# lh3/miniprot

Hardware: NVIDIA H100
Metric: proteins/s (higher is better)
Workload: dtype int16 scores

## Files before the change

miniprot_b200/csrc/cuda/chain_core.cuh:

```cuda
#pragma once
#include <stdint.h>
#include "../flagsort.hpp"

#ifdef __CUDACC__
#define CHN_HD __host__ __device__ __forceinline__
#else
#define CHN_HD inline
#endif

namespace chn {

struct Par { int32_t max_dist_x, max_dist_y, bw, max_skip, max_iter, min_cnt, min_sc; float chn_coef_log; int32_t is_spliced, kmer, bbit; };

CHN_HD Par normalise(Par p)
{
	if (p.max_dist_x < p.bw) p.max_dist_x = p.bw;
	if (p.max_dist_y < p.bw && !p.is_spliced) p.max_dist_y = p.bw;
	return p;
}

CHN_HD float log2_approx(float x)
{
	union { float f; uint32_t i; } z;
	z.f = x;
	float r = (float)((int)((z.i >> 23) & 255) - 128);
	z.i &= ~(255u << 23);
	z.i += 127u << 23;
#ifdef __CUDA_ARCH__
	float q = __fadd_rn(__fmul_rn(-0.34484843f, z.f), 2.02466578f);
	q = __fsub_rn(__fmul_rn(q, z.f), 0.67487759f);
	return __fadd_rn(r, q);
#else
	volatile float q = -0.34484843f * z.f;
	q = q + 2.02466578f;
	q = q * z.f;
	q = q - 0.67487759f;
	volatile float s = r + q;
	return s;
#endif
}

CHN_HD int32_t pair_score(const Par &p, uint64_t ai, uint64_t aj)
{
	const int32_t dq = (int32_t)ai - (int32_t)aj, dq3 = dq * 3;
	int32_t dr3, dd, dds = 0, sc;
	if (dq <= 0 || dq3 > p.max_dist_x || dq > p.max_dist_y) return INT32_MIN;
	if (p.bbit > 0) {
		const int32_t bs = 1 << p.bbit;
		dr3 = (int32_t)(((ai >> 32) - (aj >> 32)) << p.bbit);
		if (dq3 < dr3 - bs) dd = dr3 - bs - dq3, dds = -dd;
		else if (dq3 > dr3 + bs) dd = dq3 - (dr3 + bs), dds = dd;
		else dd = 0;
	} else {
		dr3 = (int32_t)((ai >> 32) - (aj >> 32));
		if (dr3 == 0) return INT32_MIN;
		dd = dr3 > dq3 ? dr3 - dq3 : dq3 - dr3;
		dds = dq3 - dr3;
	}
	if (dd > p.bw) return INT32_MIN;
	if (p.bbit > 0) sc = p.kmer < dq ? p.kmer : dq;
	else if (p.kmer <= dq && p.kmer * 3 <= dr3) sc = p.kmer;
	else {
		const int32_t dr = dr3 / 3, g = dr < dq ? dr : dq;
		sc = g < p.kmer ? g : p.kmer;
		if (dr3 - dr * 3 != 0) --sc;
	}
	if (dd > 0) {
#ifdef __CUDA_ARCH__
		const float lin = __fmul_rn((float)dd, .33334f);
		const float lg = dd >= 2 ? __fadd_rn(__fmul_rn(p.chn_coef_log, __fsub_rn(log2_approx((float)(dd + 1)), 1.0f)), 1.0f) : (float)dd;
		if (p.is_spliced && dds < 0) sc -= (int32_t)(lin < lg ? lin : lg);
		else sc -= (int32_t)__fadd_rn(lin, lg);
#else
		volatile float lin = (float)dd * .33334f;
		volatile float lg = (float)dd;
		if (dd >= 2) { volatile float t = log2_approx((float)(dd + 1)) - 1.0f; t = p.chn_coef_log * t; lg = t + 1.0f; }
		if (p.is_spliced && dds < 0) sc -= (int32_t)(lin < lg ? lin : lg);
		else { volatile float s = lin + lg; sc -= (int32_t)s; }
#endif
	}
	if (p.bbit > 0 && ai >> 32 == aj >> 32 && dd == 0) sc += 2;
	return sc;
}

CHN_HD int resolve_chunk(uint32_t rec, uint32_t skip, int32_t max_skip, int32_t &n_skip)
{
	if (skip == 0) {
		const int32_t d = (int32_t)
#ifdef __CUDA_ARCH__
			__popc(rec);
#else
			__builtin_popcount(rec);
#endif
		n_skip = n_skip > d ? n_skip - d : 0;
		return 32;
	}
	uint32_t m = rec | skip;
	while (m) {
#ifdef __CUDA_ARCH__
		const int b = __ffs(m) - 1;
#else
		const int b = __builtin_ctz(m);
#endif
		if (rec >> b & 1) { if (n_skip > 0) --n_skip; }
		else if (++n_skip > max_skip) return b;
		m &= m - 1;
	}
	return 32;
}

CHN_HD uint64_t rec_key(uint64_t r) { return r >> 32; }

template <class T, class FT, class PT>
CHN_HD int64_t bk_end(int32_t max_drop, uint64_t z, const FT *f, const PT *p, T *t)
{
	const int32_t zx = (int32_t)(z >> 32);
	int64_t i = (int64_t)(uint32_t)z, end_i = -1, max_i = i;
	int32_t max_s = 0;
	if (i < 0 || t[i] != 0) return i;
	do {
		t[i] = 2;
		end_i = i = p[i];
		const int32_t s = i < 0 ? zx : zx - (int32_t)f[i];
		if (s > max_s) max_s = s, max_i = i;
		else if (max_s - s > max_drop) break;
	} while (i >= 0 && t[i] == 0);
	for (i = (int64_t)(uint32_t)z; i >= 0 && i != end_i; i = p[i]) t[i] = 0;
	return max_i;
}

template <class T, bool PRESORTED = false, class FT = int32_t, class PT = int32_t>
CHN_HD int32_t peel_chains(const Par &p, int32_t n_z, const FT *f, const PT *pp, T *t, int32_t *v, uint64_t *z, mpb::FlagRange<uint64_t> *stack, uint64_t *u,
                           int32_t *n_v_out = 0)
{
	const int32_t max_drop = p.is_spliced ? INT32_MAX : p.bw;
	int32_t n_u = 0, n_v = 0;
	if (n_v_out) *n_v_out = 0;
	if (n_z == 0) return 0;
	if (!PRESORTED) mpb::flag_sort_by(z, z + n_z, [](const uint64_t &e) { return rec_key(e); }, stack);
	for (int32_t k = n_z - 1; k >= 0; --k) {
		const int32_t zi = (int32_t)(uint32_t)z[k], zx = (int32_t)(z[k] >> 32);
		if (zx <= p.kmer && p.min_cnt >= 2) break;
		if (t[zi] != 0) continue;
		const int32_t n_v0 = n_v;
		const int64_t end_i = bk_end(max_drop, z[k], f, pp, t);
		int64_t i;
		for (i = zi; i != end_i; i = pp[i]) v[n_v++] = (int32_t)i, t[i] = 1;
		const int32_t sc = i < 0 ? zx : zx - (int32_t)f[i];
		if (sc >= p.min_sc && n_v > n_v0 && n_v - n_v0 >= p.min_cnt) u[n_u++] = (uint64_t)sc << 32 | (uint64_t)(n_v - n_v0);
		else n_v = n_v0;
	}
	if (n_v_out) *n_v_out = n_v;
	return n_u;
}

template <class FT, class Sync>
CHN_HD void compact_chains(int32_t n_u, const uint64_t *a, FT *f, const int32_t *v, uint64_t *z, mpb::FlagRange<uint64_t> *stack, uint64_t *u, uint64_t *b,
                           int32_t *n_b_out, int lane, int n_lanes, Sync sync)
{
	if (n_u == 0) {
		if (lane == 0) *n_b_out = 0;
		return;
	}
	if (lane == 0) {
		int32_t k = 0;
		for (int32_t i = 0; i < n_u; ++i) {
			const int32_t ni = (int32_t)(uint32_t)u[i];
			z[i] = (a[v[k + ni - 1]] >> 32) << 32 | (uint32_t)i;
			f[i] = (FT)k;
			k += ni;
		}
		mpb::flag_sort_by(z, z + n_u, [](const uint64_t &e) { return rec_key(e); }, stack);
	}
	sync();
	int32_t o = 0;
	for (int32_t i = 0; i < n_u; ++i) {
		const int32_t src = (int32_t)(uint32_t)z[i], k0 = (int32_t)f[src], ni = (int32_t)(uint32_t)u[src];
		for (int32_t j = lane; j < ni; j += n_lanes) b[o + j] = a[v[k0 + (ni - j - 1)]];
		o += ni;
	}
	sync();
	for (int32_t i = lane; i < n_u; i += n_lanes) z[i] = u[(uint32_t)z[i]];
	sync();
	for (int32_t i = lane; i < n_u; i += n_lanes) u[i] = z[i];
	if (lane == 0) *n_b_out = o;
}

template <class T, bool PRESORTED = false, class FT = int32_t, class PT = int32_t>
CHN_HD int32_t peel_and_compact(const Par &p, int32_t n_z, const uint64_t *a, FT *f, const PT *pp, T *t, int32_t *v, uint64_t *z,
                                mpb::FlagRange<uint64_t> *stack, uint64_t *u, uint64_t *b, int32_t *n_b_out)
{
	const int32_t n_u = peel_chains<T, PRESORTED, FT, PT>(p, n_z, f, pp, t, v, z, stack, u);
	compact_chains(n_u, a, f, v, z, stack, u, b, n_b_out, 0, 1, [] {});
	return n_u;
}

template <class T>
CHN_HD int32_t backtrack_compact(const Par &p, int32_t n, const uint64_t *a, int32_t *f, const int32_t *pp, T *t, int32_t *v, uint64_t *z,
                                 mpb::FlagRange<uint64_t> *stack, uint64_t *u, uint64_t *b, int32_t *n_b_out)
{
	int32_t n_z = 0;
	for (int32_t i = 0; i < n; ++i) {
		t[i] = 0;
		if (f[i] >= p.min_sc) z[n_z++] = (uint64_t)(uint32_t)f[i] << 32 | (uint32_t)i;
	}
	return peel_and_compact(p, n_z, a, f, pp, t, v, z, stack, u, b, n_b_out);
}

}
```

miniprot_b200/csrc/cuda/chain_dev.hpp:

```cpp
#pragma once
#include <cuda_runtime.h>
#include <stdint.h>
#include "chain_core.cuh"

namespace mpb {
namespace cuda {

constexpr int CHAIN_STACK = 2048;

void chain_launch_fill(cudaStream_t st, const int32_t *list, const int64_t *a_off, const int32_t *cnt, const uint64_t *a, int n_prob, const chn::Par &par, int32_t *f,
                       int32_t *p, int32_t *t);
void chain_launch_smem(cudaStream_t st, const int32_t *list, int n_list, int cap, const int64_t *a_off, const int32_t *cnt, const uint64_t *a, const chn::Par &par,
                       int32_t *v, void *stack, uint64_t *u, uint64_t *b, int32_t *n_u, int32_t *n_b, int resort);
void chain_launch_bt_smem(cudaStream_t st, const int32_t *list, int n_list, int cap, const int64_t *a_off, const int32_t *cnt, const uint64_t *a, const chn::Par &par,
                          int32_t *f, const int32_t *p, int32_t *v, void *stack, uint64_t *u, uint64_t *b, int32_t *n_u, int32_t *n_b, int resort);
void chain_launch_bt(cudaStream_t st, const int32_t *list, int n_list, const int64_t *a_off, const int32_t *cnt, const uint64_t *a, const chn::Par &par, int32_t *f,
                     const int32_t *p, int32_t *t, int32_t *v, void *z, void *stack, uint64_t *u, uint64_t *b, int32_t *n_u, int32_t *n_b, int resort);

}
}
```

miniprot_b200/csrc/cuda/chain_kernels.cu:

```cuda
#include <cuda_runtime.h>
#include "chain_core.cuh"
#include "chain_dev.hpp"
#include "smem_attr.hpp"

namespace mpb {
namespace cuda {

using namespace chn;

constexpr int CHAIN_WARPS = 4;

struct AnchorBlocks {
	uint64_t prev, cur, next;
	int32_t i0;
	__device__ __forceinline__ void init(const uint64_t *a, int32_t n, int lane)
	{
		i0 = 0, prev = 0;
		cur = lane < n ? a[lane] : 0;
		next = 32 + lane < n ? a[32 + lane] : 0;
	}
	__device__ __forceinline__ void enter(const uint64_t *a, int32_t n, int32_t i, int lane)
	{
		prev = cur, cur = next, i0 = i;
		next = i + 32 + lane < n ? a[i + 32 + lane] : 0;
	}
	__device__ __forceinline__ uint64_t at(const uint64_t *a, int32_t idx) const
	{
		if (idx >= i0) return __shfl_sync(0xffffffffu, cur, idx - i0);
		if (idx >= i0 - 32) return __shfl_sync(0xffffffffu, prev, idx - (i0 - 32));
		return a[idx];
	}
	__device__ __forceinline__ uint64_t near(int32_t j) const
	{
		const uint64_t c = __shfl_sync(0xffffffffu, cur, j & 31), p = __shfl_sync(0xffffffffu, prev, j & 31);
		return j >= i0 ? c : p;
	}
};

__global__ void __launch_bounds__(CHAIN_WARPS * 32) chain_fill_kernel(const int32_t *list, const int64_t *a_off, const int32_t *cnt, const uint64_t *a_all, int n_prob, Par par,
                                                                     int32_t *f_all, int32_t *p_all, int32_t *t_all)
{
	const int warp = threadIdx.x >> 5, lane = threadIdx.x & 31;
	const int slot = blockIdx.x * CHAIN_WARPS + warp;
	if (slot >= n_prob) return;
	const int prob = list ? list[slot] : slot;
	const int64_t base = a_off[prob];
	const int32_t n = cnt ? cnt[prob] : (int32_t)(a_off[prob + 1] - base);
	const uint64_t *a = a_all + base;
	int32_t *f = f_all + base, *p = p_all + base, *t = t_all + base;
	for (int32_t i = lane; i < n; i += 32) __stcg(t + i, 0);
	__syncwarp();
	AnchorBlocks ab;
	ab.init(a, n, lane);
	int32_t fcur = 0, fprev = 0, pcur = -1, pprev = -1;
	int32_t st = 0, hi = -1, hf = 0;
	uint64_t a_hi = 0;
	for (int32_t i = 0; i < n; ++i) {
		if (i && (i & 31) == 0) ab.enter(a, n, i, lane), fprev = fcur, pprev = pcur;
		{
			const uint64_t mine = ab.cur;
			uint64_t left = __shfl_up_sync(0xffffffffu, mine, 1);
			const uint64_t last_prev = __shfl_sync(0xffffffffu, ab.prev, 31);
			if (lane == 0) left = last_prev;
			const int32_t idx = ab.i0 + lane;
			const bool iso = idx < n && (idx == 0 || (((int64_t)(mine >> 32) - (int64_t)(left >> 32)) << par.bbit) > par.max_dist_x);
			const uint32_t m = __ballot_sync(0xffffffffu, iso) >> (i & 31);
			const int run = ~m ? __ffs(~m) - 1 : 32;
			if (run > 0) {
				if (lane >= (i & 31) && lane < (i & 31) + run) {
					__stcg(f + idx, par.kmer), __stcg(p + idx, -1);
					fcur = par.kmer, pcur = -1;
				}
				i += run - 1;
				st = i, hf = par.kmer, hi = i, a_hi = __shfl_sync(0xffffffffu, mine, i & 31);
				continue;
			}
		}
		const uint64_t ai = __shfl_sync(0xffffffffu, ab.cur, i & 31);
		const int64_t xi = (int64_t)(ai >> 32);
		while (st < i && ((xi - (int64_t)(ab.at(a, st) >> 32)) << par.bbit) > par.max_dist_x) ++st;
		int32_t max_f = par.kmer, max_j = -1, n_skip = 0;
		if (hi >= 0 && hi >= st) {
			const int32_t sc = hf + pair_score(par, ai, a_hi);
			if (sc > max_f) max_f = sc, max_j = hi;
		} else hf = 0, hi = -1;
		if (i - st > par.max_iter) st = i - par.max_iter;
		bool any_mark = false;
		for (int32_t jb = i - 1; jb >= st; jb -= 32) {
			const int32_t j = jb - lane;
			const bool near = jb == i - 1;
			bool ok = j >= st;
			int32_t sc = INT32_MIN, pj = -1;
			uint64_t aj = 0;
			int32_t fj = 0;
			if (near) {
				aj = ab.near(j);
				const int32_t fc = __shfl_sync(0xffffffffu, fcur, j & 31), fp = __shfl_sync(0xffffffffu, fprev, j & 31);
				const int32_t pc = __shfl_sync(0xffffffffu, pcur, j & 31), pp = __shfl_sync(0xffffffffu, pprev, j & 31);
				fj = j >= ab.i0 ? fc : fp, pj = j >= ab.i0 ? pc : pp;
			} else if (ok) aj = a[j];
			if (ok) {
				sc = pair_score(par, ai, aj);
				ok = sc != INT32_MIN;
				if (ok) {
					if (!near) fj = __ldcg(f + j), pj = __ldcg(p + j);
					sc += fj;
				}
			}
			if (!ok) pj = -1;
			const bool mark = ok && pj >= 0;
			if (mark) __stcg(t + pj, i);
			any_mark = any_mark || __any_sync(0xffffffffu, mark);
			__syncwarp();
			const bool marked = any_mark && ok && __ldcg(t + j) == i;
			int32_t pm = ok ? sc : INT32_MIN;
#pragma unroll
			for (int d = 1; d < 32; d <<= 1) {
				const int32_t o = __shfl_up_sync(0xffffffffu, pm, d);
				if (lane >= d) pm = pm > o ? pm : o;
			}
			int32_t before = __shfl_up_sync(0xffffffffu, pm, 1);
			if (lane == 0) before = INT32_MIN;
			before = before > max_f ? before : max_f;
			const bool rec = ok && sc > before;
			const uint32_t R = __ballot_sync(0xffffffffu, rec), S = __ballot_sync(0xffffffffu, ok && !rec && marked);
			const int brk = resolve_chunk(R, S, par.max_skip, n_skip);
			const uint32_t Rb = brk >= 32 ? R : (R & ((1u << brk) - 1u));
			if (Rb) {
				const int top = 31 - __clz(Rb);
				max_f = __shfl_sync(0xffffffffu, sc, top), max_j = jb - top;
			}
			if (brk < 32) break;
		}
		if (lane == 0) __stcg(f + i, max_f), __stcg(p + i, max_j);
		if (lane == (i & 31)) fcur = max_f, pcur = max_j;
		__syncwarp();
		if (hf < max_f) hf = max_f, hi = i, a_hi = ai;
	}
}

struct WarpSortScratch { uint32_t cnt[256]; uint32_t head[256]; uint32_t tail[256]; int top; };

template <class KeyFn>
__device__ void flag_sort_warp(uint64_t *rec, int n, KeyFn key, FlagRange<uint64_t> *stack, WarpSortScratch *ws, int lane)
{
	if (n <= 64) {
		if (lane == 0) insertion_sort_by(rec, rec + n, key);
		__syncwarp();
		return;
	}
	if (lane == 0) ws->top = 1, stack[0] = FlagRange<uint64_t>{rec, rec + n, 56};
	__syncwarp();
	while (ws->top > 0) {
		const FlagRange<uint64_t> r = stack[ws->top - 1];
		__syncwarp();
		if (lane == 0) ws->top -= 1;
		const int m = (int)(r.end - r.beg);
		uint64_t lo = ~0ULL, hi = 0;
		for (int i = lane; i < m; i += 32) { const uint64_t k = key(r.beg[i]); lo = k < lo ? k : lo, hi = k > hi ? k : hi; }
		for (int d = 16; d; d >>= 1) {
			const uint64_t ol = __shfl_xor_sync(0xffffffffu, lo, d), oh = __shfl_xor_sync(0xffffffffu, hi, d);
			lo = ol < lo ? ol : lo, hi = oh > hi ? oh : hi;
		}
		int shift = r.shift;
		while (shift > 0 && (lo >> shift) == (hi >> shift)) shift -= 8;
		if (shift == 0 && lo == hi) { __syncwarp(); continue; }
		for (int k = lane; k < 256; k += 32) ws->cnt[k] = 0;
		__syncwarp();
		for (int i = lane; i < m; i += 32) atomicAdd(&ws->cnt[(key(r.beg[i]) >> shift) & 255], 1u);
		__syncwarp();
		if (lane == 0) {
			uint32_t acc = 0;
			for (int k = 0; k < 256; ++k) ws->head[k] = acc, acc += ws->cnt[k], ws->tail[k] = acc;
		}
		__syncwarp();
		{
			uint64_t *b = r.beg;
			for (int k = 0; k < 256; ++k) {
				for (;;) {
					const uint32_t h = ws->head[k], e = ws->tail[k];
					if (h >= e) break;
					const uint32_t idx = h + (uint32_t)lane;
					const bool misplaced = idx < e && (int)((key(b[idx]) >> shift) & 255) != k;
					const uint32_t mm = __ballot_sync(0xffffffffu, misplaced);
					__syncwarp();
					if (mm == 0) {
						if (lane == 0) ws->head[k] = h + 32 < e ? h + 32 : e;
						__syncwarp();
						continue;
					}
					if (lane == 0) {
						const uint32_t at = h + (uint32_t)(__ffs(mm) - 1);
						uint64_t hand = b[at];
						int d = (int)((key(hand) >> shift) & 255);
						ws->head[k] = at;
						do {
							const uint64_t next = b[ws->head[d]];
							b[ws->head[d]++] = hand;
							hand = next;
							d = (int)((key(hand) >> shift) & 255);
						} while (d != k);
						b[ws->head[k]++] = hand;
					}
					__syncwarp();
				}
			}
		}
		__syncwarp();
		if (shift > 0) {
			for (int k = lane; k < 256; k += 32) {
				const uint32_t e = ws->tail[k], bgn = k ? ws->tail[k - 1] : 0;
				if (e - bgn > 64) { const int slot = atomicAdd(&ws->top, 1); stack[slot] = FlagRange<uint64_t>{r.beg + bgn, r.beg + e, shift - 8}; }
				else if (e - bgn > 1) insertion_sort_by(r.beg + bgn, r.beg + e, key);
			}
		}
		__syncwarp();
	}
}

template <class T>
__device__ int32_t keep_filter_warp(int32_t n, int32_t n_v, const int32_t *v, T *t, const uint64_t *a, uint64_t *b, int lane)
{
	for (int32_t i = lane; i < n; i += 32) t[i] = 0;
	__syncwarp();
	for (int32_t k = lane; k < n_v; k += 32) t[v[k]] = 1;
	__syncwarp();
	int32_t o = 0;
	for (int32_t i0 = 0; i0 < n; i0 += 32) {
		const int32_t i = i0 + lane;
		const bool keep = i < n && t[i] != 0;
		const uint32_t m = __ballot_sync(0xffffffffu, keep);
		if (keep) b[o + __popc(m & ((1u << lane) - 1u))] = a[i];
		o += __popc(m);
	}
	return o;
}

__global__ void __launch_bounds__(32) chain_smem_kernel(const int32_t *list, int n_list, int cap, const int64_t *a_off, const int32_t *cnt, const uint64_t *a_all,
                                                       Par par, int32_t *v_all, FlagRange<uint64_t> *stack_all, uint64_t *u_all, uint64_t *b_all,
                                                       int32_t *n_u_out, int32_t *n_b_out, int resort)
{
	extern __shared__ uint64_t zs[];
	__shared__ WarpSortScratch ws;
	if ((int)blockIdx.x >= n_list) return;
	const int prob = list[blockIdx.x], lane = threadIdx.x;
	const int64_t base = a_off[prob];
	const int32_t n = cnt ? cnt[prob] : (int32_t)(a_off[prob + 1] - base);
	const uint64_t *a = a_all + base;
	int32_t *f = (int32_t*)(zs + cap);
	int16_t *p = (int16_t*)(f + cap), *t = p + cap;
	for (int32_t i = lane; i < n; i += 32) t[i] = 0;
	__syncwarp();
	AnchorBlocks ab;
	ab.init(a, n, lane);
	int32_t st = 0, hi = -1, hf = 0;
	uint64_t a_hi = 0;
	for (int32_t i = 0; i < n; ++i) {
		if (i && (i & 31) == 0) ab.enter(a, n, i, lane);
		{
			const uint64_t mine = ab.cur;
			uint64_t left = __shfl_up_sync(0xffffffffu, mine, 1);
			const uint64_t last_prev = __shfl_sync(0xffffffffu, ab.prev, 31);
			if (lane == 0) left = last_prev;
			const int32_t idx = ab.i0 + lane;
			const bool iso = idx < n && (idx == 0 || (((int64_t)(mine >> 32) - (int64_t)(left >> 32)) << par.bbit) > par.max_dist_x);
			const uint32_t m = __ballot_sync(0xffffffffu, iso) >> (i & 31);
			const int run = ~m ? __ffs(~m) - 1 : 32;
			if (run > 0) {
				if (lane >= (i & 31) && lane < (i & 31) + run) f[idx] = par.kmer, p[idx] = -1;
				__syncwarp();
				i += run - 1;
				st = i, hf = par.kmer, hi = i, a_hi = __shfl_sync(0xffffffffu, mine, i & 31);
				continue;
			}
		}
		const uint64_t ai = __shfl_sync(0xffffffffu, ab.cur, i & 31);
		const int64_t xi = (int64_t)(ai >> 32);
		while (st < i && ((xi - (int64_t)(ab.at(a, st) >> 32)) << par.bbit) > par.max_dist_x) ++st;
		int32_t max_f = par.kmer, max_j = -1, n_skip = 0;
		if (hi >= 0 && hi >= st) {
			const int32_t sc = hf + pair_score(par, ai, a_hi);
			if (sc > max_f) max_f = sc, max_j = hi;
		} else hf = 0, hi = -1;
		if (i - st > par.max_iter) st = i - par.max_iter;
		for (int32_t jb = i - 1; jb >= st; jb -= 32) {
			const int32_t j = jb - lane;
			bool ok = j >= st;
			int32_t sc = INT32_MIN, pj = -1;
			uint64_t aj = 0;
			if (jb == i - 1) aj = ab.near(j);
			else if (ok) aj = a[j];
			if (ok) {
				sc = pair_score(par, ai, aj);
				ok = sc != INT32_MIN;
				if (ok) sc += f[j], pj = p[j];
			}
			if (ok && pj >= 0) t[pj] = (int16_t)i;
			__syncwarp();
			const bool marked = ok && t[j] == (int16_t)i;
			int32_t pm = ok ? sc : INT32_MIN;
#pragma unroll
			for (int d = 1; d < 32; d <<= 1) {
				const int32_t o = __shfl_up_sync(0xffffffffu, pm, d);
				if (lane >= d) pm = pm > o ? pm : o;
			}
			int32_t before = __shfl_up_sync(0xffffffffu, pm, 1);
			if (lane == 0) before = INT32_MIN;
			before = before > max_f ? before : max_f;
			const bool rec = ok && sc > before;
			const uint32_t R = __ballot_sync(0xffffffffu, rec), S = __ballot_sync(0xffffffffu, ok && !rec && marked);
			const int brk = resolve_chunk(R, S, par.max_skip, n_skip);
			const uint32_t Rb = brk >= 32 ? R : (R & ((1u << brk) - 1u));
			if (Rb) {
				const int top = 31 - __clz(Rb);
				max_f = __shfl_sync(0xffffffffu, sc, top), max_j = jb - top;
			}
			if (brk < 32) break;
		}
		if (lane == 0) f[i] = max_f, p[i] = (int16_t)max_j;
		__syncwarp();
		if (hf < max_f) hf = max_f, hi = i, a_hi = ai;
	}
	int32_t n_z = 0;
	for (int32_t i0 = 0; i0 < n; i0 += 32) {
		const int32_t i = i0 + lane;
		const bool keep = i < n && f[i] >= par.min_sc;
		if (i < n) t[i] = 0;
		const uint32_t m = __ballot_sync(0xffffffffu, keep);
		if (keep) zs[n_z + __popc(m & ((1u << lane) - 1u))] = (uint64_t)(uint32_t)f[i] << 32 | (uint32_t)i;
		n_z += __popc(m);
	}
	__syncwarp();
	int32_t n_u = 0, n_b = 0;
	FlagRange<uint64_t> *stack = stack_all + (int64_t)prob * CHAIN_STACK;
	flag_sort_warp(zs, n_z, [](const uint64_t &e) { return rec_key(e); }, stack, &ws, lane);
	int32_t n_v = 0;
	if (lane == 0 && n > 0) n_u = peel_chains<int16_t, true, int32_t, int16_t>(par, n_z, f, p, t, v_all + base, zs, stack, u_all + base, &n_v);
	n_u = __shfl_sync(0xffffffffu, n_u, 0), n_v = __shfl_sync(0xffffffffu, n_v, 0);
	__syncwarp();
	if (resort) n_b = keep_filter_warp(n, n_v, v_all + base, t, a, b_all + base, lane);
	else {
		if (n > 0) compact_chains(n_u, a, f, v_all + base, zs, stack, u_all + base, b_all + base, &n_b, lane, 32, [] { __syncwarp(); });
		__syncwarp();
		n_b = __shfl_sync(0xffffffffu, n_b, 0);
	}
	if (lane == 0) n_u_out[prob] = n_u, n_b_out[prob] = n_b;
}

__global__ void __launch_bounds__(32) chain_bt_smem_kernel(const int32_t *list, int n_list, int cap, const int64_t *a_off, const int32_t *cnt, const uint64_t *a_all,
                                                          Par par, int32_t *f_all, const int32_t *p_all, int32_t *v_all, FlagRange<uint64_t> *stack_all,
                                                          uint64_t *u_all, uint64_t *b_all, int32_t *n_u_out, int32_t *n_b_out, int resort)
{
	extern __shared__ uint64_t zs[];
	__shared__ WarpSortScratch ws;
	if ((int)blockIdx.x >= n_list) return;
	const int prob = list[blockIdx.x], lane = threadIdx.x;
	const int64_t base = a_off[prob];
	const int32_t n = cnt ? cnt[prob] : (int32_t)(a_off[prob + 1] - base);
	uint16_t *fs = (uint16_t*)(zs + cap);
	int16_t *ps = (int16_t*)(fs + cap);
	int8_t *ts = (int8_t*)(ps + cap);
	int32_t *fg = f_all + base;
	const int32_t *pg = p_all + base;
	int32_t n_z = 0;
	bool wide = false;
	for (int32_t i0 = 0; i0 < n; i0 += 32) {
		const int32_t i = i0 + lane;
		const int32_t fi = i < n ? fg[i] : 0;
		const bool keep = i < n && fi >= par.min_sc;
		if (i < n) ts[i] = 0, ps[i] = (int16_t)pg[i], fs[i] = (uint16_t)fi;
		wide |= fi > 65535;
		const uint32_t m = __ballot_sync(0xffffffffu, keep);
		if (keep) zs[n_z + __popc(m & ((1u << lane) - 1u))] = (uint64_t)(uint32_t)fi << 32 | (uint32_t)i;
		n_z += __popc(m);
	}
	wide = __any_sync(0xffffffffu, wide);
	__syncwarp();
	int32_t n_u = 0, n_b = 0;
	FlagRange<uint64_t> *stack = stack_all + (int64_t)prob * CHAIN_STACK;
	int32_t *v = v_all + base;
	uint64_t *u = u_all + base, *b = b_all + base;
	flag_sort_warp(zs, n_z, [](const uint64_t &e) { return rec_key(e); }, stack, &ws, lane);
	int32_t n_v = 0;
	if (lane == 0 && n > 0) {
		if (!wide) n_u = peel_chains<int8_t, true, uint16_t, int16_t>(par, n_z, fs, ps, ts, v, zs, stack, u, &n_v);
		else n_u = peel_chains<int8_t, true, int32_t, int16_t>(par, n_z, fg, ps, ts, v, zs, stack, u, &n_v);
	}
	n_u = __shfl_sync(0xffffffffu, n_u, 0), n_v = __shfl_sync(0xffffffffu, n_v, 0);
	__syncwarp();
	if (resort) n_b = keep_filter_warp(n, n_v, v, ts, a_all + base, b, lane);
	else {
		if (n > 0) {
			if (!wide) compact_chains(n_u, a_all + base, fs, v, zs, stack, u, b, &n_b, lane, 32, [] { __syncwarp(); });
			else compact_chains(n_u, a_all + base, fg, v, zs, stack, u, b, &n_b, lane, 32, [] { __syncwarp(); });
		}
		__syncwarp();
		n_b = __shfl_sync(0xffffffffu, n_b, 0);
	}
	if (lane == 0) n_u_out[prob] = n_u, n_b_out[prob] = n_b;
}

__global__ void __launch_bounds__(32) chain_bt_global_kernel(const int32_t *list, int n_list, const int64_t *a_off, const int32_t *cnt, const uint64_t *a_all, Par par,
                                                            int32_t *f_all, const int32_t *p_all, int32_t *t_all, int32_t *v_all, uint64_t *z_all,
                                                            FlagRange<uint64_t> *stack_all, uint64_t *u_all, uint64_t *b_all, int32_t *n_u_out, int32_t *n_b_out, int resort)
{
	__shared__ WarpSortScratch ws;
	if ((int)blockIdx.x >= n_list) return;
	const int prob = list[blockIdx.x], lane = threadIdx.x;
	const int64_t base = a_off[prob];
	const int32_t n = cnt ? cnt[prob] : (int32_t)(a_off[prob + 1] - base);
	int32_t *f = f_all + base, *t = t_all + base, *v = v_all + base;
	const int32_t *pp = p_all + base;
	uint64_t *z = z_all + base, *u = u_all + base, *b = b_all + base;
	const uint64_t *a = a_all + base;
	int32_t n_z = 0;
	for (int32_t i0 = 0; i0 < n; i0 += 32) {
		const int32_t i = i0 + lane;
		const int32_t fi = i < n ? __ldcg(f + i) : 0;
		const bool keep = i < n && fi >= par.min_sc;
		if (i < n) t[i] = 0;
		const uint32_t m = __ballot_sync(0xffffffffu, keep);
		if (keep) z[n_z + __popc(m & ((1u << lane) - 1u))] = (uint64_t)(uint32_t)fi << 32 | (uint32_t)i;
		n_z += __popc(m);
	}
	__syncwarp();
	int32_t n_u = 0, n_b = 0, n_v = 0;
	FlagRange<uint64_t> *stack = stack_all + (int64_t)prob * CHAIN_STACK;
	flag_sort_warp(z, n_z, [](const uint64_t &e) { return rec_key(e); }, stack, &ws, lane);
	if (lane == 0 && n > 0) n_u = peel_chains<int32_t, true, int32_t, int32_t>(par, n_z, f, pp, t, v, z, stack, u, &n_v);
	n_u = __shfl_sync(0xffffffffu, n_u, 0), n_v = __shfl_sync(0xffffffffu, n_v, 0);
	__syncwarp();
	if (resort) n_b = keep_filter_warp(n, n_v, v, t, a, b, lane);
	else {
		if (n > 0) compact_chains(n_u, a, f, v, z, stack, u, b, &n_b, lane, 32, [] { __syncwarp(); });
		__syncwarp();
		n_b = __shfl_sync(0xffffffffu, n_b, 0);
	}
	if (lane == 0) n_u_out[prob] = n_u, n_b_out[prob] = n_b;
}

void chain_launch_fill(cudaStream_t st, const int32_t *list, const int64_t *a_off, const int32_t *cnt, const uint64_t *a, int n_prob, const Par &par, int32_t *f, int32_t *p,
                       int32_t *t)
{
	if (n_prob > 0) chain_fill_kernel<<<(n_prob + CHAIN_WARPS - 1) / CHAIN_WARPS, CHAIN_WARPS * 32, 0, st>>>(list, a_off, cnt, a, n_prob, par, f, p, t);
}

void chain_launch_smem(cudaStream_t st, const int32_t *list, int n_list, int cap, const int64_t *a_off, const int32_t *cnt, const uint64_t *a, const Par &par, int32_t *v,
                       void *stack, uint64_t *u, uint64_t *b, int32_t *n_u, int32_t *n_b, int resort)
{
	if (n_list <= 0) return;
	const int smem = cap * 16 + 16;
	static SmemLimit lim;
	lim.raise(chain_smem_kernel, smem);
	chain_smem_kernel<<<n_list, 32, smem, st>>>(list, n_list, cap, a_off, cnt, a, par, v, (FlagRange<uint64_t>*)stack, u, b, n_u, n_b, resort);
}

void chain_launch_bt_smem(cudaStream_t st, const int32_t *list, int n_list, int cap, const int64_t *a_off, const int32_t *cnt, const uint64_t *a, const Par &par,
                          int32_t *f, const int32_t *p, int32_t *v, void *stack, uint64_t *u, uint64_t *b, int32_t *n_u, int32_t *n_b, int resort)
{
	if (n_list <= 0) return;
	const int smem = cap * 13 + 16;
	static SmemLimit lim;
	lim.raise(chain_bt_smem_kernel, smem);
	chain_bt_smem_kernel<<<n_list, 32, smem, st>>>(list, n_list, cap, a_off, cnt, a, par, f, p, v, (FlagRange<uint64_t>*)stack, u, b, n_u, n_b, resort);
}

void chain_launch_bt(cudaStream_t st, const int32_t *list, int n_list, const int64_t *a_off, const int32_t *cnt, const uint64_t *a, const Par &par, int32_t *f,
                     const int32_t *p, int32_t *t, int32_t *v, void *z, void *stack, uint64_t *u, uint64_t *b, int32_t *n_u, int32_t *n_b, int resort)
{
	if (n_list > 0)
		chain_bt_global_kernel<<<n_list, 32, 0, st>>>(list, n_list, a_off, cnt, a, par, f, p, t, v, (uint64_t*)z, (FlagRange<uint64_t>*)stack, u, b, n_u, n_b, resort);
}

}
}
```

miniprot_b200/csrc/cuda/stage_host.cu:

```cuda
#include <algorithm>
#include <numeric>
#include "ctx.hpp"
#include "stages_dev.hpp"
#include "chain_dev.hpp"
#include "seed_dev.hpp"
#include "../slices.hpp"

namespace mpb {
namespace cuda {

__global__ void gather_u64_kernel(const uint64_t *src, const int64_t *src_off, const int32_t *cnt, uint64_t *dst, const int64_t *dst_off, int n_seg)
{
	const int s = blockIdx.x;
	if (s >= n_seg) return;
	const uint64_t *from = src + src_off[s];
	uint64_t *to = dst + dst_off[s];
	for (int i = threadIdx.x; i < cnt[s]; i += blockDim.x) to[i] = from[i];
}

static void fill_seed_const(const mp_idx_t *mi, const mp_mapopt_t *opt, SeedConst &c)
{
	memcpy(c.aa13, ns_tab_aa13, 256);
	memcpy(c.codon, ns_tab_codon, 64);
	memcpy(c.codon13, ns_tab_codon13, 64);
	c.kmer = mi->opt.kmer, c.mod_bit = mi->opt.mod_bit, c.max_occ = opt->max_occ, c.n_kb = mi->n_kb;
}

static chn::Par chain_par(int32_t mdx, int32_t mdy, int32_t bw, const mp_mapopt_t *o, int32_t min_cnt, int32_t min_sc, int32_t kmer, int32_t bbit)
{
	chn::Par p;
	p.max_dist_x = mdx, p.max_dist_y = mdy, p.bw = bw, p.max_skip = o->max_chn_max_skip, p.max_iter = o->max_chn_iter, p.min_cnt = min_cnt, p.min_sc = min_sc;
	p.chn_coef_log = o->chn_coef_log, p.is_spliced = !(o->flag & MP_F_NO_SPLICE), p.kmer = kmer, p.bbit = bbit;
	return chn::normalise(p);
}

struct Carver {
	char *base;
	size_t used = 0;
	explicit Carver(void *p) : base((char*)p) {}
	template <class T> T *take(size_t n) { used = (used + 255) & ~(size_t)255; T *r = (T*)(base + used); used += sizeof(T) * n; return r; }
};
template <class F> static size_t carve_size(F f) { Carver c(0); f(c); return c.used + 256; }

struct ChainScratch {
	int32_t *f, *p, *t, *v, *d_nu, *d_nb, *d_nu2, *d_nb2, *d_list;
	uint64_t *z, *du, *db, *du2, *db2, *gu, *gb;
	int64_t *d_go_u, *d_go_b;
	void *stack;
	void layout(Carver &c, int n_prob, size_t N)
	{
		f = c.take<int32_t>(N + 1), p = c.take<int32_t>(N + 1), t = c.take<int32_t>(N + 1), v = c.take<int32_t>(N + 1);
		z = c.take<uint64_t>(N + 1);
		d_list = c.take<int32_t>((size_t)n_prob);
		du = c.take<uint64_t>(N + 1), db = c.take<uint64_t>(N + 1), du2 = c.take<uint64_t>(N + 1), db2 = c.take<uint64_t>(N + 1);
		gu = c.take<uint64_t>(N + 1), gb = c.take<uint64_t>(N + 1);
		d_nu = c.take<int32_t>((size_t)n_prob), d_nb = c.take<int32_t>((size_t)n_prob), d_nu2 = c.take<int32_t>((size_t)n_prob), d_nb2 = c.take<int32_t>((size_t)n_prob);
		d_go_u = c.take<int64_t>((size_t)n_prob + 1), d_go_b = c.take<int64_t>((size_t)n_prob + 1);
		stack = c.take<char>((size_t)n_prob * CHAIN_STACK * 24);
	}
	static size_t bytes(int n_prob, size_t N) { ChainScratch s; return carve_size([&](Carver &c) { s.layout(c, n_prob, N); }); }
};

static const int64_t kAnchorBytesChain = 88, kAnchorBytesSeed = 16, kProbBytes = (int64_t)CHAIN_STACK * 24 + 128, kSliceFixed = (int64_t)64 << 10;

static inline size_t anchor_arena(size_t N) { return sizeof(uint64_t) * (N + 2); }

static int64_t plan_items(mpb_ctx_s *ctx, std::initializer_list<DevBuf*> mine, std::initializer_list<size_t> whole, int n, const int64_t *cnt, int64_t per_anchor,
                          SlicePlan &p, int64_t &n_slices)
{
	int64_t room = -1;
	if (ctx->mem.budget == 0 && Ledger::fits(mine, whole)) {
		p.cut.assign(1, 0), p.cut.push_back(n), p.n_over = 0;
	} else {
		std::vector<int64_t> bytes((size_t)n);
		for (int i = 0; i < n; ++i) bytes[(size_t)i] = cnt[i] * per_anchor + kProbBytes;
		room = ctx->mem.plan(mine, [&](int64_t r) {
			plan_slices(n, bytes.data(), cnt, kSliceFixed, r / 5 * 4, kSliceMaxCount, p);
			int64_t most = 0;
			for (int k = 0; k < p.n_slices(); ++k) {
				int64_t s = kSliceFixed;
				for (int i = p.cut[(size_t)k]; i < p.cut[(size_t)k + 1]; ++i) s += bytes[(size_t)i];
				most = std::max(most, s);
			}
			return most / 4 * 5;
		});
	}
	n_slices += p.n_slices(), ctx->mem.n_over_budget += p.n_over;
	return room;
}

static void chain_problems(mpb_ctx_s *ctx, int n_prob, const std::vector<int64_t> &h_off, const int64_t *d_off, uint64_t *d_a, const chn::Par *pre, const chn::Par &mainp,
                           std::vector<int32_t> &n_u, std::vector<int32_t> &n_b, std::vector<uint64_t> &u, std::vector<uint64_t> &bb)
{
	cudaStream_t st = ctx->stream;
	const size_t N = (size_t)h_off[(size_t)n_prob];
	n_u.assign((size_t)n_prob, 0), n_b.assign((size_t)n_prob, 0), u.clear(), bb.clear();
	if (n_prob == 0) return;
	ChainScratch cs;
	ctx->b_c[8].reserve(ChainScratch::bytes(n_prob, N));
	Carver cv(ctx->b_c[8].p);
	cs.layout(cv, n_prob, N);
	int32_t *f = cs.f, *p = cs.p, *t = cs.t, *v = cs.v, *d_nu = cs.d_nu, *d_nb = cs.d_nb, *d_nu2 = cs.d_nu2, *d_nb2 = cs.d_nb2, *d_list = cs.d_list;
	uint64_t *z = cs.z, *du = cs.du, *db = cs.db, *du2 = cs.du2, *db2 = cs.db2, *gu = cs.gu, *gb = cs.gb;
	int64_t *d_go_u = cs.d_go_u, *d_go_b = cs.d_go_b;
	void *stack = cs.stack;
	static const int NC = 11;
	static const int caps[NC] = { 2048, 3072, 4096, 5120, 6144, 7168, 8192, 10240, 12288, 14000, 16384 };
	static const int fused_max = getenv("MPB_CHAIN_FUSED_MAX") ? atoi(getenv("MPB_CHAIN_FUSED_MAX")) : 2048;
	std::vector<int32_t> lists[NC + 1], flat, sizes((size_t)n_prob);
	size_t lfirst[NC + 1];
	for (int i = 0; i < n_prob; ++i) sizes[(size_t)i] = (int32_t)(h_off[(size_t)i + 1] - h_off[(size_t)i]);
	auto classify = [&]() {
		flat.clear();
		for (int c = 0; c <= NC; ++c) lists[c].clear();
		for (int i = 0; i < n_prob; ++i) {
			const int32_t n = sizes[(size_t)i];
			int c = 0;
			while (c < NC && n > caps[c]) ++c;
			lists[c].push_back(i);
		}
		for (int c = 0; c <= NC; ++c) lfirst[c] = flat.size(), flat.insert(flat.end(), lists[c].begin(), lists[c].end());
		MPB_CUDA_OK(cudaMemcpyAsync(d_list, flat.data(), sizeof(int32_t) * flat.size(), cudaMemcpyHostToDevice, st));
	};
	classify();
	auto chain_once = [&](const int32_t *cnt, const uint64_t *in, const chn::Par &par, uint64_t *uo, uint64_t *bo, int32_t *nuo, int32_t *nbo, int resort) {
		MPB_CUDA_OK(cudaEventRecord(ctx->ev_fork, st));
		for (int c = NC; c >= 0; --c) {
			if (lists[c].empty()) continue;
			cudaStream_t ss = ctx->side[c];
			const int32_t *lst = d_list + lfirst[c];
			const int nl = (int)lists[c].size();
			MPB_CUDA_OK(cudaStreamWaitEvent(ss, ctx->ev_fork, 0));
			if (c < NC && caps[c] <= fused_max) {
				chain_launch_smem(ss, lst, nl, caps[c], d_off, cnt, in, par, v, stack, uo, bo, nuo, nbo, resort);
				ctx->stats.kernel_launches += 1;
			} else {
				chain_launch_fill(ss, lst, d_off, cnt, in, nl, par, f, p, t);
				if (c < NC) chain_launch_bt_smem(ss, lst, nl, caps[c], d_off, cnt, in, par, f, p, v, stack, uo, bo, nuo, nbo, resort);
				else chain_launch_bt(ss, lst, nl, d_off, cnt, in, par, f, p, t, v, z, stack, uo, bo, nuo, nbo, resort);
				ctx->stats.kernel_launches += 2;
			}
			MPB_CUDA_OK(cudaEventRecord(ctx->ev_join[c], ss));
			MPB_CUDA_OK(cudaStreamWaitEvent(st, ctx->ev_join[c], 0));
		}
	};
	ctx->time_begin();
	const uint64_t *in = d_a;
	const int32_t *cnt = 0;
	if (pre) {
		chain_once(0, d_a, *pre, du, db, d_nu, d_nb, 1);
		in = db, cnt = d_nb;
		MPB_CUDA_OK(cudaMemcpyAsync(sizes.data(), d_nb, sizeof(int32_t) * (size_t)n_prob, cudaMemcpyDeviceToHost, st));
		MPB_CUDA_OK(cudaStreamSynchronize(st));
		classify();
	}
	chain_once(cnt, in, mainp, du2, db2, d_nu2, d_nb2, 0);
	MPB_CUDA_OK(cudaMemcpyAsync(n_u.data(), d_nu2, sizeof(int32_t) * (size_t)n_prob, cudaMemcpyDeviceToHost, st));
	MPB_CUDA_OK(cudaMemcpyAsync(n_b.data(), d_nb2, sizeof(int32_t) * (size_t)n_prob, cudaMemcpyDeviceToHost, st));
	MPB_CUDA_OK(cudaStreamSynchronize(st));
	std::vector<int64_t> go_u((size_t)n_prob + 1, 0), go_b((size_t)n_prob + 1, 0);
	for (int i = 0; i < n_prob; ++i) go_u[(size_t)i + 1] = go_u[(size_t)i] + n_u[(size_t)i], go_b[(size_t)i + 1] = go_b[(size_t)i] + n_b[(size_t)i];
	MPB_CUDA_OK(cudaMemcpyAsync(d_go_u, go_u.data(), sizeof(int64_t) * go_u.size(), cudaMemcpyHostToDevice, st));
	MPB_CUDA_OK(cudaMemcpyAsync(d_go_b, go_b.data(), sizeof(int64_t) * go_b.size(), cudaMemcpyHostToDevice, st));
	gather_u64_kernel<<<n_prob, 128, 0, st>>>(du2, d_off, d_nu2, gu, d_go_u, n_prob);
	gather_u64_kernel<<<n_prob, 128, 0, st>>>(db2, d_off, d_nb2, gb, d_go_b, n_prob);
	ctx->stats.kernel_launches += 2;
	u.resize((size_t)go_u.back()), bb.resize((size_t)go_b.back());
	if (!u.empty()) MPB_CUDA_OK(cudaMemcpyAsync(u.data(), gu, sizeof(uint64_t) * u.size(), cudaMemcpyDeviceToHost, st));
	if (!bb.empty()) MPB_CUDA_OK(cudaMemcpyAsync(bb.data(), gb, sizeof(uint64_t) * bb.size(), cudaMemcpyDeviceToHost, st));
	ctx->stats.ms_chain += ctx->time_end();
	MPB_CUDA_OK(cudaGetLastError());
	ctx->stats.d2h_bytes += (int64_t)(sizeof(uint64_t) * (u.size() + bb.size()) + 8 * (size_t)n_prob);
	ctx->stats.n_chain_problems += n_prob * (pre ? 2 : 1);
}

void chain_batch_run(mpb_ctx_s *ctx, const chn::Par &par, int n_prob, const int64_t *a_off, const uint64_t *a, std::vector<int32_t> &n_u, std::vector<int32_t> &n_b,
                     std::vector<uint64_t> &u, std::vector<uint64_t> &bb)
{
	cudaStream_t st = ctx->stream;
	Busy busy({ &ctx->b_c[1], &ctx->b_c[7], &ctx->b_c[8] });
	std::vector<int64_t> off(a_off, a_off + n_prob + 1);
	const size_t N = (size_t)off[(size_t)n_prob];
	ctx->b_c[1].reserve(sizeof(uint64_t) * (N + 2));
	ctx->b_c[7].reserve(sizeof(int64_t) * ((size_t)n_prob + 2));
	MPB_CUDA_OK(cudaMemcpyAsync(ctx->b_c[1].p, a, sizeof(uint64_t) * N, cudaMemcpyHostToDevice, st));
	MPB_CUDA_OK(cudaMemcpyAsync(ctx->b_c[7].p, off.data(), sizeof(int64_t) * off.size(), cudaMemcpyHostToDevice, st));
	ctx->stats.h2d_bytes += (int64_t)(sizeof(uint64_t) * N);
	chain_problems(ctx, n_prob, off, ctx->b_c[7].as<int64_t>(), ctx->b_c[1].as<uint64_t>(), 0, chn::normalise(par), n_u, n_b, u, bb);
}

template <class F>
static void seed_run(mpb_ctx_s *ctx, const mp_idx_t *mi, int32_t max_occ, const Batch &b, const std::vector<int32_t> &aa_off, const char *d_aa, bool chain, F fn)
{
	cudaStream_t st = ctx->stream;
	const int n_q = b.n;
	const size_t R = (size_t)aa_off[(size_t)n_q];
	Busy busy({ &ctx->b_aa, &ctx->b_c[0], &ctx->b_c[1], &ctx->b_c[2], &ctx->b_c[3], &ctx->b_c[8] });
	ClaimScope claim(ctx->mem);
	SeedConst cst;
	mp_mapopt_t tmp;
	memset(&tmp, 0, sizeof(tmp));
	tmp.max_occ = max_occ;
	fill_seed_const(mi, &tmp, cst);
	int32_t *d_aa_off, *sd_pos, *d_nsd;
	uint32_t *sd_hash;
	int64_t *sd_cnt, *sd_aoff, *d_tot, *d_a_off;
	auto layout = [&](Carver &c) {
		d_aa_off = c.take<int32_t>((size_t)n_q + 1), sd_hash = c.take<uint32_t>(R + 1), sd_pos = c.take<int32_t>(R + 1);
		sd_cnt = c.take<int64_t>(R + 1), sd_aoff = c.take<int64_t>(R + 1), d_nsd = c.take<int32_t>((size_t)n_q), d_tot = c.take<int64_t>((size_t)n_q);
		d_a_off = c.take<int64_t>((size_t)n_q + 1);
	};
	ctx->b_c[0].reserve(carve_size(layout));
	Carver cv(ctx->b_c[0].p);
	layout(cv);
	MPB_CUDA_OK(cudaMemcpyAsync(d_aa_off, aa_off.data(), sizeof(int32_t) * ((size_t)n_q + 1), cudaMemcpyHostToDevice, st));
	ctx->time_begin();
	seed_launch_sketch(st, d_aa, d_aa_off, n_q, cst, ctx->d_ki, sd_hash, sd_pos, sd_cnt, sd_aoff, d_nsd, d_tot);
	std::vector<int64_t> tot((size_t)n_q);
	MPB_CUDA_OK(cudaMemcpyAsync(tot.data(), d_tot, sizeof(int64_t) * (size_t)n_q, cudaMemcpyDeviceToHost, st));
	ctx->stats.ms_seed += ctx->time_end();
	ctx->stats.kernel_launches += 1;
	const size_t N_all = (size_t)std::accumulate(tot.begin(), tot.end(), (int64_t)0);
	SlicePlan plan;
	const int64_t room = plan_items(ctx, { &ctx->b_c[1], &ctx->b_c[2], &ctx->b_c[8] },
	                                { anchor_arena(N_all), anchor_arena(N_all), chain ? ChainScratch::bytes(n_q, N_all) : 0 }, n_q, tot.data(),
	                                chain ? kAnchorBytesChain : kAnchorBytesSeed, plan, ctx->mem.n_slices_seed);
	std::vector<int64_t> a_off;
	for (int k = 0; k < plan.n_slices(); ++k) {
		const int q0 = plan.cut[(size_t)k], n = plan.cut[(size_t)k + 1] - q0;
		a_off.assign((size_t)n + 1, 0);
		for (int q = 0; q < n; ++q) a_off[(size_t)q + 1] = a_off[(size_t)q] + tot[(size_t)(q0 + q)];
		const size_t N = (size_t)a_off[(size_t)n];
		if (room >= 0) ctx->mem.trim({ &ctx->b_c[1], &ctx->b_c[2], &ctx->b_c[8] }, { anchor_arena(N), anchor_arena(N), chain ? ChainScratch::bytes(n, N) : 0 }, room);
		ctx->time_begin();
		MPB_CUDA_OK(cudaMemcpyAsync(d_a_off, a_off.data(), sizeof(int64_t) * a_off.size(), cudaMemcpyHostToDevice, st));
		ctx->b_c[1].reserve(anchor_arena(N));
		ctx->b_c[2].reserve(anchor_arena(N));
		uint64_t *d_a = ctx->b_c[1].as<uint64_t>(), *d_tmp = ctx->b_c[2].as<uint64_t>();
		seed_launch_expand(st, d_aa_off + q0, n, ctx->d_ki, ctx->d_kb, sd_hash, sd_pos, sd_cnt, sd_aoff, d_nsd + q0, d_a_off, d_a);
		seg_sort_u64(ctx, st, d_a, d_tmp, n, a_off.data(), a_off.data() + 1);
		ctx->stats.ms_seed += ctx->time_end();
		ctx->stats.kernel_launches += 2;
		ctx->stats.n_anchors += (int64_t)N;
		fn(q0, q0 + n, a_off, (const int64_t*)d_a_off, d_a);
	}
}

static void append_anchors(mpb_ctx_s *ctx, int q0, const std::vector<int64_t> &a_off, const uint64_t *d_a, std::vector<int64_t> &off, std::vector<uint64_t> &a)
{
	const int n = (int)a_off.size() - 1;
	const size_t at = a.size();
	a.resize(at + (size_t)a_off[(size_t)n]);
	if (a.size() > at) MPB_CUDA_OK(cudaMemcpyAsync(a.data() + at, d_a, sizeof(uint64_t) * (a.size() - at), cudaMemcpyDeviceToHost, ctx->stream));
	MPB_CUDA_OK(cudaStreamSynchronize(ctx->stream));
	ctx->stats.d2h_bytes += (int64_t)(sizeof(uint64_t) * (a.size() - at));
	for (int q = 0; q < n; ++q) off[(size_t)(q0 + q) + 1] = off[(size_t)q0] + a_off[(size_t)q + 1];
}

void seed_batch_run(mpb_ctx_s *ctx, const mp_idx_t *mi, int32_t max_occ, const Batch &b, const std::vector<int32_t> &aa_off, const char *d_aa,
                    std::vector<int64_t> &a_off, std::vector<uint64_t> &a)
{
	a_off.assign((size_t)b.n + 1, 0), a.clear();
	if (b.n == 0) return;
	seed_run(ctx, mi, max_occ, b, aa_off, d_aa, false, [&](int q0, int, const std::vector<int64_t> &so, const int64_t *, uint64_t *d_a) {
		append_anchors(ctx, q0, so, d_a, a_off, a);
	});
}

static void chain_seeds(mpb_ctx_s *ctx, const mp_idx_t *mi, const mp_mapopt_t *opt, int q0, const std::vector<int64_t> &a_off, const int64_t *d_a_off, uint64_t *d_a,
                        ChainSet &out)
{
	const int n = (int)a_off.size() - 1;
	const int32_t w = 1 << mi->opt.bbit, spl = !(opt->flag & MP_F_NO_SPLICE);
	const chn::Par pre = chain_par(w, w, w, opt, 2, 0, mi->opt.kmer, mi->opt.bbit);
	const chn::Par mainp = chain_par(opt->max_intron, opt->max_gap, opt->bw, opt, opt->min_chn_cnt, opt->min_chn_sc, mi->opt.kmer, mi->opt.bbit);
	std::vector<int32_t> n_u, n_b;
	std::vector<uint64_t> u, bb;
	chain_problems(ctx, n, a_off, d_a_off, d_a, (!(opt->flag & MP_F_NO_PRE_CHAIN) && spl) ? &pre : 0, mainp, n_u, n_b, u, bb);
	for (int q = 0; q < n; ++q) {
		const size_t g = (size_t)(q0 + q);
		out.u_off[g + 1] = out.u_off[g] + n_u[(size_t)q], out.a_off[g + 1] = out.a_off[g] + n_b[(size_t)q];
	}
	if (out.u.empty()) out.u.swap(u); else out.u.insert(out.u.end(), u.begin(), u.end());
	if (out.a.empty()) out.a.swap(bb); else out.a.insert(out.a.end(), bb.begin(), bb.end());
}

void seed_chain_run(mpb_ctx_s *ctx, const mp_idx_t *mi, const mp_mapopt_t *opt, const Batch &b, const std::vector<int32_t> &aa_off, const char *d_aa, ChainSet &out)
{
	const int n_q = b.n;
	out.u_off.assign((size_t)n_q + 1, 0), out.a_off.assign((size_t)n_q + 1, 0), out.u.clear(), out.a.clear();
	if (n_q == 0) return;
	if (out.want_seeds) out.seed_off.assign((size_t)n_q + 1, 0), out.seed.clear();
	seed_run(ctx, mi, opt->max_occ, b, aa_off, d_aa, true, [&](int q0, int, const std::vector<int64_t> &a_off, const int64_t *d_a_off, uint64_t *d_a) {
		if (out.want_seeds) append_anchors(ctx, q0, a_off, d_a, out.seed_off, out.seed);
		chain_seeds(ctx, mi, opt, q0, a_off, d_a_off, d_a, out);
	});
}

template <class F>
static void seed_loci_run(mpb_ctx_s *ctx, const mp_idx_t *vi, int32_t max_occ, const Batch &b, const std::vector<int32_t> &aa_off, const char *d_aa, bool chain, F fn)
{
	cudaStream_t st = ctx->stream;
	const int n_q = b.n;
	const size_t R = (size_t)aa_off[(size_t)n_q];
	Busy busy({ &ctx->b_aa, &ctx->b_c[0], &ctx->b_c[1], &ctx->b_c[2], &ctx->b_c[3], &ctx->b_c[4], &ctx->b_c[5], &ctx->b_c[6], &ctx->b_c[8] });
	ClaimScope claim(ctx->mem);
	SeedConst cst;
	mp_mapopt_t tmp;
	memset(&tmp, 0, sizeof(tmp));
	tmp.max_occ = max_occ;
	fill_seed_const(vi, &tmp, cst);
	std::vector<LocusStrand> strands((size_t)n_q * 2);
	std::vector<LocusUnit> units;
	std::vector<size_t> unit_first((size_t)n_q + 1, 0);
	for (int q = 0; q < n_q; ++q) {
		const mp_ctg_t *c = &vi->nt->ctg[q];
		for (int s = 0; s < 2; ++s) {
			LocusStrand &ls = strands[(size_t)q * 2 + s];
			ls.g_start = s ? c->off + c->len - 1 : c->off, ls.dir = s ? -1 : 1, ls.comp = s, ls.len = c->len, ls.boff = vi->bo[q * 2 + s], ls.qid = q;
			const int64_t step = (int64_t)WIN_TILE * 16;
			for (int64_t p = 0; p < c->len; p += step) units.push_back(LocusUnit{ q * 2 + s, 0, p, std::min(p + step, (int64_t)c->len) });
		}
		unit_first[(size_t)q + 1] = units.size();
	}
	const int n_units = (int)units.size();
	int32_t *d_aa_off, *d_npk, *sd_pos;
	uint32_t *sd_idx;
	uint64_t *d_pk, *d_pk_tmp;
	int64_t *sd_lo, *sd_cnt, *sd_aoff, *d_unit_off, *d_unit_n, *d_seg, *d_nu, *d_tot, *d_a_off;
	LocusUnit *d_units;
	LocusStrand *d_strands;
	auto layout = [&](Carver &c) {
		d_aa_off = c.take<int32_t>((size_t)n_q + 1), d_npk = c.take<int32_t>((size_t)n_q), d_pk = c.take<uint64_t>(R + 1), d_pk_tmp = c.take<uint64_t>(R + 1);
		sd_idx = c.take<uint32_t>(R + 1), sd_pos = c.take<int32_t>(R + 1), sd_lo = c.take<int64_t>(R + 1), sd_cnt = c.take<int64_t>(R + 1), sd_aoff = c.take<int64_t>(R + 1);
		d_units = c.take<LocusUnit>((size_t)n_units + 1), d_strands = c.take<LocusStrand>(strands.size());
		d_unit_off = c.take<int64_t>((size_t)n_units + 1), d_unit_n = c.take<int64_t>((size_t)n_units + 1);
		d_seg = c.take<int64_t>((size_t)n_q + 1), d_nu = c.take<int64_t>((size_t)n_q), d_tot = c.take<int64_t>((size_t)n_q), d_a_off = c.take<int64_t>((size_t)n_q + 1);
	};
	ctx->b_c[0].reserve(carve_size(layout));
	Carver cv(ctx->b_c[0].p);
	layout(cv);
	MPB_CUDA_OK(cudaMemcpyAsync(d_aa_off, aa_off.data(), sizeof(int32_t) * ((size_t)n_q + 1), cudaMemcpyHostToDevice, st));
	if (n_units) MPB_CUDA_OK(cudaMemcpyAsync(d_units, units.data(), sizeof(LocusUnit) * units.size(), cudaMemcpyHostToDevice, st));
	MPB_CUDA_OK(cudaMemcpyAsync(d_strands, strands.data(), sizeof(LocusStrand) * strands.size(), cudaMemcpyHostToDevice, st));
	ctx->stats.h2d_bytes += (int64_t)(sizeof(LocusUnit) * units.size() + sizeof(LocusStrand) * strands.size());
	ctx->time_begin();
	seed_launch_prot_kmer(st, d_aa, d_aa_off, n_q, cst, cst.kmer, cst.mod_bit, d_pk, d_npk);
	std::vector<int32_t> n_pk((size_t)n_q);
	MPB_CUDA_OK(cudaMemcpyAsync(n_pk.data(), d_npk, sizeof(int32_t) * (size_t)n_q, cudaMemcpyDeviceToHost, st));
	MPB_CUDA_OK(cudaStreamSynchronize(st));
	{
		std::vector<int64_t> sb((size_t)n_q), se((size_t)n_q);
		for (int q = 0; q < n_q; ++q) sb[(size_t)q] = aa_off[(size_t)q], se[(size_t)q] = aa_off[(size_t)q] + n_pk[(size_t)q];
		seg_sort_u64(ctx, st, d_pk, d_pk_tmp, n_q, sb.data(), se.data());
	}
	locus_launch_join(st, false, d_units, n_units, d_strands, ctx->d_seq, cst, vi->opt.min_aa_len, vi->opt.bbit, d_pk, d_aa_off, d_npk, 0, d_unit_n, 0);
	std::vector<int64_t> unit_n((size_t)n_units + 1, 0), m_q((size_t)n_q, 0);
	if (n_units) MPB_CUDA_OK(cudaMemcpyAsync(unit_n.data(), d_unit_n, sizeof(int64_t) * (size_t)n_units, cudaMemcpyDeviceToHost, st));
	ctx->stats.ms_seed += ctx->time_end();
	ctx->stats.kernel_launches += 2;
	for (int q = 0; q < n_q; ++q)
		for (size_t u = unit_first[(size_t)q]; u < unit_first[(size_t)q + 1]; ++u) m_q[(size_t)q] += unit_n[u];
	const size_t M_all = (size_t)std::accumulate(m_q.begin(), m_q.end(), (int64_t)0);
	SlicePlan outer;
	const int64_t room_p = plan_items(ctx, { &ctx->b_c[4], &ctx->b_c[5], &ctx->b_c[6] }, { anchor_arena(M_all), anchor_arena(M_all), sizeof(uint32_t) * (M_all + 2) }, n_q,
	                                  m_q.data(), 20 * 4, outer, ctx->mem.n_slices_loci);
	const int64_t per_anchor = chain ? kAnchorBytesChain : kAnchorBytesSeed;
	std::vector<int64_t> unit_off, seg, tot, a_off;
	for (int k = 0; k < outer.n_slices(); ++k) {
		const int p0 = outer.cut[(size_t)k], np = outer.cut[(size_t)k + 1] - p0;
		const size_t u0 = unit_first[(size_t)p0], nu = unit_first[(size_t)(p0 + np)] - u0;
		unit_off.assign(nu + 1, 0), seg.assign((size_t)np + 1, 0);
		for (size_t u = 0; u < nu; ++u) unit_off[u + 1] = unit_off[u] + unit_n[u0 + u];
		for (int q = 0; q <= np; ++q) seg[(size_t)q] = unit_off[unit_first[(size_t)(p0 + q)] - u0];
		const size_t M = (size_t)seg[(size_t)np];
		if (room_p >= 0) ctx->mem.trim({ &ctx->b_c[4], &ctx->b_c[5], &ctx->b_c[6] }, { anchor_arena(M), anchor_arena(M), sizeof(uint32_t) * (M + 2) }, room_p);
		ctx->time_begin();
		MPB_CUDA_OK(cudaMemcpyAsync(d_unit_off, unit_off.data(), sizeof(int64_t) * unit_off.size(), cudaMemcpyHostToDevice, st));
		MPB_CUDA_OK(cudaMemcpyAsync(d_seg, seg.data(), sizeof(int64_t) * seg.size(), cudaMemcpyHostToDevice, st));
		ctx->b_c[4].reserve(anchor_arena(M)), ctx->b_c[5].reserve(anchor_arena(M)), ctx->b_c[6].reserve(sizeof(uint32_t) * (M + 2));
		uint64_t *d_pairs = ctx->b_c[4].as<uint64_t>(), *d_uniq = ctx->b_c[5].as<uint64_t>();
		uint32_t *d_blk = ctx->b_c[6].as<uint32_t>();
		locus_launch_join(st, true, d_units + u0, (int)nu, d_strands, ctx->d_seq, cst, vi->opt.min_aa_len, vi->opt.bbit, d_pk, d_aa_off, d_npk, d_unit_off, 0, d_pairs);
		seg_sort_u64(ctx, st, d_pairs, d_uniq, np, seg.data(), seg.data() + 1);
		locus_launch_unique(st, d_pairs, d_seg, np, d_uniq, d_blk, d_nu + p0);
		locus_launch_occ(st, d_pk, d_aa_off + p0, d_npk + p0, np, d_uniq, d_seg, d_nu + p0, max_occ, sd_idx, sd_pos, sd_lo, sd_cnt, sd_aoff, d_tot + p0);
		tot.assign((size_t)np, 0);
		MPB_CUDA_OK(cudaMemcpyAsync(tot.data(), d_tot + p0, sizeof(int64_t) * (size_t)np, cudaMemcpyDeviceToHost, st));
		ctx->stats.ms_seed += ctx->time_end();
		ctx->stats.kernel_launches += 3;
		const size_t N_all = (size_t)std::accumulate(tot.begin(), tot.end(), (int64_t)0);
		SlicePlan inner;
		const int64_t room = plan_items(ctx, { &ctx->b_c[1], &ctx->b_c[2], &ctx->b_c[8] },
		                                { anchor_arena(N_all), anchor_arena(N_all), chain ? ChainScratch::bytes(np, N_all) : 0 }, np, tot.data(), per_anchor, inner,
		                                ctx->mem.n_slices_loci);
		ctx->mem.n_slices_loci -= 1;
		for (int j = 0; j < inner.n_slices(); ++j) {
			const int r0 = inner.cut[(size_t)j], n = inner.cut[(size_t)j + 1] - r0;
			a_off.assign((size_t)n + 1, 0);
			for (int q = 0; q < n; ++q) a_off[(size_t)q + 1] = a_off[(size_t)q] + tot[(size_t)(r0 + q)];
			const size_t N = (size_t)a_off[(size_t)n];
			if (room >= 0) ctx->mem.trim({ &ctx->b_c[1], &ctx->b_c[2], &ctx->b_c[8] }, { anchor_arena(N), anchor_arena(N), chain ? ChainScratch::bytes(n, N) : 0 }, room);
			ctx->time_begin();
			MPB_CUDA_OK(cudaMemcpyAsync(d_a_off, a_off.data(), sizeof(int64_t) * a_off.size(), cudaMemcpyHostToDevice, st));
			ctx->b_c[1].reserve(anchor_arena(N));
			ctx->b_c[2].reserve(anchor_arena(N));
			uint64_t *d_a = ctx->b_c[1].as<uint64_t>(), *d_tmp = ctx->b_c[2].as<uint64_t>();
			const int q0 = p0 + r0;
			seed_launch_expand(st, d_aa_off + q0, n, sd_lo, d_blk, sd_idx, sd_pos, sd_cnt, sd_aoff, d_npk + q0, d_a_off, d_a);
			seg_sort_u64(ctx, st, d_a, d_tmp, n, a_off.data(), a_off.data() + 1);
			ctx->stats.ms_seed += ctx->time_end();
			MPB_CUDA_OK(cudaGetLastError());
			ctx->stats.kernel_launches += 1;
			ctx->stats.n_anchors += (int64_t)N;
			fn(q0, q0 + n, a_off, (const int64_t*)d_a_off, d_a);
		}
	}
}

void seed_chain_loci_run(mpb_ctx_s *ctx, const mp_idx_t *vi, const mp_mapopt_t *opt, const Batch &b, const std::vector<int32_t> &aa_off, const char *d_aa, ChainSet &out)
{
	const int n_q = b.n;
	out.u_off.assign((size_t)n_q + 1, 0), out.a_off.assign((size_t)n_q + 1, 0), out.u.clear(), out.a.clear();
	if (n_q == 0) return;
	seed_loci_run(ctx, vi, opt->max_occ, b, aa_off, d_aa, true, [&](int q0, int, const std::vector<int64_t> &a_off, const int64_t *d_a_off, uint64_t *d_a) {
		chain_seeds(ctx, vi, opt, q0, a_off, d_a_off, d_a, out);
	});
}

void seed_loci_batch_run(mpb_ctx_s *ctx, const mp_idx_t *vi, int32_t max_occ, const Batch &b, const std::vector<int32_t> &aa_off, const char *d_aa,
                         std::vector<int64_t> &a_off, std::vector<uint64_t> &a)
{
	a_off.assign((size_t)b.n + 1, 0), a.clear();
	if (b.n == 0) return;
	seed_loci_run(ctx, vi, max_occ, b, aa_off, d_aa, false, [&](int q0, int, const std::vector<int64_t> &so, const int64_t *, uint64_t *d_a) {
		append_anchors(ctx, q0, so, d_a, a_off, a);
	});
}

void refine_run(mpb_ctx_s *ctx, const mp_idx_t *mi, const mp_mapopt_t *opt, const Batch &b, const std::vector<int32_t> &aa_off, const char *d_aa,
                const std::vector<RefineJob> &jobs, RefineSet &out)
{
	cudaStream_t st = ctx->stream;
	const int n_q = b.n, n_j = (int)jobs.size();
	const size_t R = (size_t)aa_off[(size_t)n_q];
	out.off.assign((size_t)n_j + 1, 0), out.a.clear(), out.sc.assign((size_t)n_j, 0);
	if (n_j == 0) return;
	if (mi->opt.min_aa_len > WIN_MAX_MIN_AA) { fprintf(stderr, "[miniprot_b200] min ORF length %d > %d is not supported by the window kernel\n", mi->opt.min_aa_len, WIN_MAX_MIN_AA); abort(); }
	Busy busy({ &ctx->b_aa, &ctx->b_c[3], &ctx->b_c[4], &ctx->b_c[5], &ctx->b_c[6], &ctx->b_c[8] });
	ClaimScope claim(ctx->mem);
	SeedConst cst;
	fill_seed_const(mi, opt, cst);
	const int k2 = opt->kmer2;
	std::vector<int32_t> n_pk((size_t)n_q);
	std::vector<int64_t> seg_b((size_t)n_q), seg_e((size_t)n_q);
	std::vector<WinJob> wj((size_t)n_j);
	int64_t grp_tot = 0;
	int32_t *d_aa_off, *d_npk, *d_grp;
	uint64_t *d_pk, *d_pk_tmp;
	int64_t *d_seg_b, *d_seg_e, *d_na, *d_a_off;
	WinJob *d_wj;
	for (int j = 0; j < n_j; ++j) grp_tot += b.len[jobs[(size_t)j].qid] + 1;
	auto layout = [&](Carver &c) {
		d_aa_off = c.take<int32_t>((size_t)n_q + 1), d_npk = c.take<int32_t>((size_t)n_q), d_pk = c.take<uint64_t>(R + 1), d_pk_tmp = c.take<uint64_t>(R + 1);
		d_seg_b = c.take<int64_t>((size_t)n_q), d_seg_e = c.take<int64_t>((size_t)n_q), d_wj = c.take<WinJob>((size_t)n_j), d_grp = c.take<int32_t>((size_t)grp_tot + 1);
		d_na = c.take<int64_t>((size_t)n_j), d_a_off = c.take<int64_t>((size_t)n_j + 1);
	};
	ctx->b_c[4].reserve(carve_size(layout));
	Carver cv(ctx->b_c[4].p);
	layout(cv);
	MPB_CUDA_OK(cudaMemcpyAsync(d_aa_off, aa_off.data(), sizeof(int32_t) * ((size_t)n_q + 1), cudaMemcpyHostToDevice, st));
	ctx->time_begin();
	seed_launch_prot_kmer(st, d_aa, d_aa_off, n_q, cst, k2, 0, d_pk, d_npk);
	MPB_CUDA_OK(cudaMemcpyAsync(n_pk.data(), d_npk, sizeof(int32_t) * (size_t)n_q, cudaMemcpyDeviceToHost, st));
	MPB_CUDA_OK(cudaStreamSynchronize(st));
	for (int q = 0; q < n_q; ++q) seg_b[(size_t)q] = aa_off[(size_t)q], seg_e[(size_t)q] = aa_off[(size_t)q] + n_pk[(size_t)q];
	MPB_CUDA_OK(cudaMemcpyAsync(d_seg_b, seg_b.data(), sizeof(int64_t) * (size_t)n_q, cudaMemcpyHostToDevice, st));
	MPB_CUDA_OK(cudaMemcpyAsync(d_seg_e, seg_e.data(), sizeof(int64_t) * (size_t)n_q, cudaMemcpyHostToDevice, st));
	seg_sort_u64(ctx, st, d_pk, d_pk_tmp, n_q, seg_b.data(), seg_e.data());
	int64_t go = 0;
	for (int j = 0; j < n_j; ++j) {
		const RefineJob &r = jobs[(size_t)j];
		const mp_ctg_t *c = &mi->nt->ctg[r.vid >> 1];
		WinJob &w = wj[(size_t)j];
		const bool rev = r.vid & 1;
		w.g_start = rev ? c->off + c->len - 1 - r.as : c->off + r.as, w.dir = rev ? -1 : 1, w.comp = rev ? 1 : 0;
		w.len = r.ae - r.as, w.qid = r.qid, w.pad_ = 0, w.grp_off = go;
		go += b.len[r.qid] + 1;
	}
	MPB_CUDA_OK(cudaMemcpyAsync(d_wj, wj.data(), sizeof(WinJob) * (size_t)n_j, cudaMemcpyHostToDevice, st));
	win_launch_count(st, d_wj, n_j, ctx->d_seq, cst, k2, mi->opt.min_aa_len, opt->max_ava, d_pk, d_aa_off, d_npk, d_grp, d_na);
	std::vector<int64_t> na((size_t)n_j), a_off;
	MPB_CUDA_OK(cudaMemcpyAsync(na.data(), d_na, sizeof(int64_t) * (size_t)n_j, cudaMemcpyDeviceToHost, st));
	ctx->stats.ms_refine += ctx->time_end();
	ctx->stats.kernel_launches += 3;
	ctx->stats.n_refine_regions += n_j;
	const chn::Par par = chain_par(opt->max_intron, opt->max_gap, opt->bw, opt, opt->min_chn_cnt, opt->min_chn_sc, k2, 0);
	const size_t N_all = (size_t)std::accumulate(na.begin(), na.end(), (int64_t)0);
	SlicePlan plan;
	const int64_t room = plan_items(ctx, { &ctx->b_c[5], &ctx->b_c[6], &ctx->b_c[8] }, { anchor_arena(N_all), anchor_arena(N_all), ChainScratch::bytes(n_j, N_all) }, n_j,
	                                na.data(), kAnchorBytesChain, plan, ctx->mem.n_slices_refine);
	std::vector<int32_t> n_u, n_b;
	std::vector<uint64_t> u, bb;
	for (int k = 0; k < plan.n_slices(); ++k) {
		const int j0 = plan.cut[(size_t)k], n = plan.cut[(size_t)k + 1] - j0;
		a_off.assign((size_t)n + 1, 0);
		for (int j = 0; j < n; ++j) a_off[(size_t)j + 1] = a_off[(size_t)j] + na[(size_t)(j0 + j)];
		const size_t N = (size_t)a_off[(size_t)n];
		if (room >= 0) ctx->mem.trim({ &ctx->b_c[5], &ctx->b_c[6], &ctx->b_c[8] }, { anchor_arena(N), anchor_arena(N), ChainScratch::bytes(n, N) }, room);
		ctx->time_begin();
		MPB_CUDA_OK(cudaMemcpyAsync(d_a_off, a_off.data(), sizeof(int64_t) * a_off.size(), cudaMemcpyHostToDevice, st));
		ctx->b_c[5].reserve(anchor_arena(N));
		ctx->b_c[6].reserve(anchor_arena(N));
		uint64_t *d_a = ctx->b_c[5].as<uint64_t>(), *d_tmp = ctx->b_c[6].as<uint64_t>();
		win_launch_emit(st, d_wj + j0, n, ctx->d_seq, cst, k2, mi->opt.min_aa_len, d_pk, d_aa_off, d_npk, d_grp, d_a_off, d_a);
		seg_sort_u64(ctx, st, d_a, d_tmp, n, a_off.data(), a_off.data() + 1);
		ctx->stats.ms_refine += ctx->time_end();
		ctx->stats.kernel_launches += 2;
		chain_problems(ctx, n, a_off, d_a_off, d_a, 0, par, n_u, n_b, u, bb);
		size_t uo = 0, bo = 0;
		for (int j = 0; j < n; ++j) {
			const int32_t nu = n_u[(size_t)j];
			if (nu > 0) {
				int32_t best = 0, mx = (int32_t)(u[uo] >> 32);
				for (int32_t i = 1; i < nu; ++i) if (mx < (int32_t)(u[uo + (size_t)i] >> 32)) mx = (int32_t)(u[uo + (size_t)i] >> 32), best = i;
				size_t kk = 0;
				for (int32_t i = 0; i < best; ++i) kk += (uint32_t)u[uo + (size_t)i];
				const uint32_t cnt = (uint32_t)u[uo + (size_t)best];
				out.a.insert(out.a.end(), bb.begin() + (ptrdiff_t)(bo + kk), bb.begin() + (ptrdiff_t)(bo + kk + cnt));
				out.sc[(size_t)(j0 + j)] = mx;
			}
			out.off[(size_t)(j0 + j) + 1] = (int64_t)out.a.size();
			uo += (size_t)nu, bo += (size_t)n_b[(size_t)j];
		}
	}
}

}
}
```

Measured before the change: 19890.

## Split chain DP fill into independent segments processed per-lane or per-warp

Replaces the single-warp-per-problem chaining fill (and the fused small-problem smem kernel) with a block-per-problem kernel. The kernel first detects isolated anchors and segment starts, then has warps claim segments dynamically. Short segments run serially per lane in shared memory, and long segments run warp-parallel in shared or global memory. The aim is to expose more parallelism within large problems and cut wasted work on sparse anchors. It also batches the compaction loop and adds optional trace timing, at the cost of an extra kernel per class for small problems and more shared memory.

```diff
diff --git a/miniprot_b200/csrc/cuda/chain_core.cuh b/miniprot_b200/csrc/cuda/chain_core.cuh
--- a/miniprot_b200/csrc/cuda/chain_core.cuh
+++ b/miniprot_b200/csrc/cuda/chain_core.cuh
@@ -81,6 +81,44 @@
 	}
 	if (p.bbit > 0 && ai >> 32 == aj >> 32 && dd == 0) sc += 2;
 	return sc;
+}
+
+CHN_HD bool isolated(const Par &p, uint64_t aprev, uint64_t ai)
+{
+	return (((int64_t)(ai >> 32) - (int64_t)(aprev >> 32)) << p.bbit) > p.max_dist_x;
+}
+
+template <class FT, class PT, class TT>
+CHN_HD void fill_serial(const Par &par, const uint64_t *a, int32_t n, FT *f, PT *p, TT *t)
+{
+	for (int32_t i = 0; i < n; ++i) t[i] = 0;
+	int32_t st = 0, hi = 0, hf = par.kmer;
+	f[0] = (FT)par.kmer, p[0] = (PT)-1;
+	for (int32_t i = 1; i < n; ++i) {
+		const uint64_t ai = a[i];
+		const int64_t xi = (int64_t)(ai >> 32);
+		while (st < i && ((xi - (int64_t)(a[st] >> 32)) << par.bbit) > par.max_dist_x) ++st;
+		int32_t max_f = par.kmer, max_j = -1, n_skip = 0;
+		if (hi >= 0 && hi >= st) {
+			const int32_t sc = hf + pair_score(par, ai, a[hi]);
+			if (sc > max_f) max_f = sc, max_j = hi;
+		} else hf = 0, hi = -1;
+		if (i - st > par.max_iter) st = i - par.max_iter;
+		for (int32_t j = i - 1; j >= st; --j) {
+			int32_t sc = pair_score(par, ai, a[j]);
+			if (sc == INT32_MIN) continue;
+			sc += (int32_t)f[j];
+			if (sc > max_f) {
+				max_f = sc, max_j = j;
+				if (n_skip > 0) --n_skip;
+			} else if ((int32_t)t[j] == i) {
+				if (++n_skip > par.max_skip) break;
+			}
+			if (p[j] >= 0) t[p[j]] = (TT)i;
+		}
+		f[i] = (FT)max_f, p[i] = (PT)max_j;
+		if (hf < max_f) hf = max_f, hi = i;
+	}
 }
 
 CHN_HD int resolve_chunk(uint32_t rec, uint32_t skip, int32_t max_skip, int32_t &n_skip)
diff --git a/miniprot_b200/csrc/cuda/chain_dev.hpp b/miniprot_b200/csrc/cuda/chain_dev.hpp
--- a/miniprot_b200/csrc/cuda/chain_dev.hpp
+++ b/miniprot_b200/csrc/cuda/chain_dev.hpp
@@ -8,10 +8,10 @@
 
 constexpr int CHAIN_STACK = 2048;
 
-void chain_launch_fill(cudaStream_t st, const int32_t *list, const int64_t *a_off, const int32_t *cnt, const uint64_t *a, int n_prob, const chn::Par &par, int32_t *f,
-                       int32_t *p, int32_t *t);
-void chain_launch_smem(cudaStream_t st, const int32_t *list, int n_list, int cap, const int64_t *a_off, const int32_t *cnt, const uint64_t *a, const chn::Par &par,
-                       int32_t *v, void *stack, uint64_t *u, uint64_t *b, int32_t *n_u, int32_t *n_b, int resort);
+constexpr int SEG_POOL = 2048;
+
+void chain_launch_fill(cudaStream_t st, const int32_t *list, int n_list, int pool, const int64_t *a_off, const int32_t *cnt, const uint64_t *a, const chn::Par &par,
+                       int32_t *f, int32_t *p, int32_t *t, int32_t *seg, int32_t *stat);
 void chain_launch_bt_smem(cudaStream_t st, const int32_t *list, int n_list, int cap, const int64_t *a_off, const int32_t *cnt, const uint64_t *a, const chn::Par &par,
                           int32_t *f, const int32_t *p, int32_t *v, void *stack, uint64_t *u, uint64_t *b, int32_t *n_u, int32_t *n_b, int resort);
 void chain_launch_bt(cudaStream_t st, const int32_t *list, int n_list, const int64_t *a_off, const int32_t *cnt, const uint64_t *a, const chn::Par &par, int32_t *f,
diff --git a/miniprot_b200/csrc/cuda/chain_kernels.cu b/miniprot_b200/csrc/cuda/chain_kernels.cu
--- a/miniprot_b200/csrc/cuda/chain_kernels.cu
+++ b/miniprot_b200/csrc/cuda/chain_kernels.cu
@@ -8,77 +8,46 @@
 
 using namespace chn;
 
-constexpr int CHAIN_WARPS = 4;
-
-struct AnchorBlocks {
-	uint64_t prev, cur, next;
-	int32_t i0;
-	__device__ __forceinline__ void init(const uint64_t *a, int32_t n, int lane)
-	{
-		i0 = 0, prev = 0;
-		cur = lane < n ? a[lane] : 0;
-		next = 32 + lane < n ? a[32 + lane] : 0;
-	}
-	__device__ __forceinline__ void enter(const uint64_t *a, int32_t n, int32_t i, int lane)
-	{
-		prev = cur, cur = next, i0 = i;
-		next = i + 32 + lane < n ? a[i + 32 + lane] : 0;
-	}
-	__device__ __forceinline__ uint64_t at(const uint64_t *a, int32_t idx) const
-	{
-		if (idx >= i0) return __shfl_sync(0xffffffffu, cur, idx - i0);
-		if (idx >= i0 - 32) return __shfl_sync(0xffffffffu, prev, idx - (i0 - 32));
-		return a[idx];
-	}
-	__device__ __forceinline__ uint64_t near(int32_t j) const
-	{
-		const uint64_t c = __shfl_sync(0xffffffffu, cur, j & 31), p = __shfl_sync(0xffffffffu, prev, j & 31);
-		return j >= i0 ? c : p;
-	}
+constexpr int SEG_WARPS = 4, SEG_SHORT = 16;
+static_assert(SEG_POOL / SEG_WARPS >= 32 * SEG_SHORT, "a warp's slice holds a short segment per lane");
+
+struct SegShared {
+	const uint64_t *as;
+	int32_t *fs;
+	int16_t *ps, *ts;
+	int32_t *fg, *pg;
+	int32_t s0;
+	__device__ __forceinline__ uint64_t a(int32_t j) const { return as[j]; }
+	__device__ __forceinline__ int32_t f(int32_t j) const { return fs[j]; }
+	__device__ __forceinline__ int32_t p(int32_t j) const { return ps[j]; }
+	__device__ __forceinline__ void mark(int32_t j, int32_t i) const { ts[j] = (int16_t)i; }
+	__device__ __forceinline__ bool marked(int32_t j, int32_t i) const { return ts[j] == (int16_t)i; }
+	__device__ __forceinline__ void put(int32_t i, int32_t fi, int32_t pi) const { fs[i] = fi, ps[i] = (int16_t)pi, fg[i] = fi, pg[i] = pi < 0 ? -1 : s0 + pi; }
 };
 
-__global__ void __launch_bounds__(CHAIN_WARPS * 32) chain_fill_kernel(const int32_t *list, const int64_t *a_off, const int32_t *cnt, const uint64_t *a_all, int n_prob, Par par,
-                                                                     int32_t *f_all, int32_t *p_all, int32_t *t_all)
-{
-	const int warp = threadIdx.x >> 5, lane = threadIdx.x & 31;
-	const int slot = blockIdx.x * CHAIN_WARPS + warp;
-	if (slot >= n_prob) return;
-	const int prob = list ? list[slot] : slot;
-	const int64_t base = a_off[prob];
-	const int32_t n = cnt ? cnt[prob] : (int32_t)(a_off[prob + 1] - base);
-	const uint64_t *a = a_all + base;
-	int32_t *f = f_all + base, *p = p_all + base, *t = t_all + base;
-	for (int32_t i = lane; i < n; i += 32) __stcg(t + i, 0);
-	__syncwarp();
-	AnchorBlocks ab;
-	ab.init(a, n, lane);
-	int32_t fcur = 0, fprev = 0, pcur = -1, pprev = -1;
-	int32_t st = 0, hi = -1, hf = 0;
-	uint64_t a_hi = 0;
-	for (int32_t i = 0; i < n; ++i) {
-		if (i && (i & 31) == 0) ab.enter(a, n, i, lane), fprev = fcur, pprev = pcur;
-		{
-			const uint64_t mine = ab.cur;
-			uint64_t left = __shfl_up_sync(0xffffffffu, mine, 1);
-			const uint64_t last_prev = __shfl_sync(0xffffffffu, ab.prev, 31);
-			if (lane == 0) left = last_prev;
-			const int32_t idx = ab.i0 + lane;
-			const bool iso = idx < n && (idx == 0 || (((int64_t)(mine >> 32) - (int64_t)(left >> 32)) << par.bbit) > par.max_dist_x);
-			const uint32_t m = __ballot_sync(0xffffffffu, iso) >> (i & 31);
-			const int run = ~m ? __ffs(~m) - 1 : 32;
-			if (run > 0) {
-				if (lane >= (i & 31) && lane < (i & 31) + run) {
-					__stcg(f + idx, par.kmer), __stcg(p + idx, -1);
-					fcur = par.kmer, pcur = -1;
-				}
-				i += run - 1;
-				st = i, hf = par.kmer, hi = i, a_hi = __shfl_sync(0xffffffffu, mine, i & 31);
-				continue;
-			}
-		}
-		const uint64_t ai = __shfl_sync(0xffffffffu, ab.cur, i & 31);
+struct SegGlobal {
+	const uint64_t *ag;
+	int32_t *fg, *pg, *tg;
+	int32_t s0;
+	__device__ __forceinline__ uint64_t a(int32_t j) const { return __ldg(ag + j); }
+	__device__ __forceinline__ int32_t f(int32_t j) const { return __ldcg(fg + j); }
+	__device__ __forceinline__ int32_t p(int32_t j) const { const int32_t v = __ldcg(pg + j); return v < 0 ? -1 : v - s0; }
+	__device__ __forceinline__ void mark(int32_t j, int32_t i) const { __stcg(tg + j, i); }
+	__device__ __forceinline__ bool marked(int32_t j, int32_t i) const { return __ldcg(tg + j) == i; }
+	__device__ __forceinline__ void put(int32_t i, int32_t fi, int32_t pi) const { __stcg(fg + i, fi), __stcg(pg + i, pi < 0 ? -1 : s0 + pi); }
+};
+
+template <class S>
+__device__ void fill_warp(const Par &par, int32_t n, const S &s, int lane)
+{
+	int32_t st = 0, hi = 0, hf = par.kmer;
+	uint64_t a_hi = s.a(0);
+	if (lane == 0) s.put(0, par.kmer, -1);
+	__syncwarp();
+	for (int32_t i = 1; i < n; ++i) {
+		const uint64_t ai = s.a(i);
 		const int64_t xi = (int64_t)(ai >> 32);
-		while (st < i && ((xi - (int64_t)(ab.at(a, st) >> 32)) << par.bbit) > par.max_dist_x) ++st;
+		while (st < i && ((xi - (int64_t)(s.a(st) >> 32)) << par.bbit) > par.max_dist_x) ++st;
 		int32_t max_f = par.kmer, max_j = -1, n_skip = 0;
 		if (hi >= 0 && hi >= st) {
 			const int32_t sc = hf + pair_score(par, ai, a_hi);
@@ -88,31 +57,18 @@
 		bool any_mark = false;
 		for (int32_t jb = i - 1; jb >= st; jb -= 32) {
 			const int32_t j = jb - lane;
-			const bool near = jb == i - 1;
 			bool ok = j >= st;
 			int32_t sc = INT32_MIN, pj = -1;
-			uint64_t aj = 0;
-			int32_t fj = 0;
-			if (near) {
-				aj = ab.near(j);
-				const int32_t fc = __shfl_sync(0xffffffffu, fcur, j & 31), fp = __shfl_sync(0xffffffffu, fprev, j & 31);
-				const int32_t pc = __shfl_sync(0xffffffffu, pcur, j & 31), pp = __shfl_sync(0xffffffffu, pprev, j & 31);
-				fj = j >= ab.i0 ? fc : fp, pj = j >= ab.i0 ? pc : pp;
-			} else if (ok) aj = a[j];
 			if (ok) {
-				sc = pair_score(par, ai, aj);
+				sc = pair_score(par, ai, s.a(j));
 				ok = sc != INT32_MIN;
-				if (ok) {
-					if (!near) fj = __ldcg(f + j), pj = __ldcg(p + j);
-					sc += fj;
-				}
-			}
-			if (!ok) pj = -1;
+				if (ok) sc += s.f(j), pj = s.p(j);
+			}
 			const bool mark = ok && pj >= 0;
-			if (mark) __stcg(t + pj, i);
+			if (mark) s.mark(pj, i);
 			any_mark = any_mark || __any_sync(0xffffffffu, mark);
 			__syncwarp();
-			const bool marked = any_mark && ok && __ldcg(t + j) == i;
+			const bool marked = any_mark && ok && s.marked(j, i);
 			int32_t pm = ok ? sc : INT32_MIN;
 #pragma unroll
 			for (int d = 1; d < 32; d <<= 1) {
@@ -132,12 +88,101 @@
 			}
 			if (brk < 32) break;
 		}
-		if (lane == 0) __stcg(f + i, max_f), __stcg(p + i, max_j);
-		if (lane == (i & 31)) fcur = max_f, pcur = max_j;
+		if (lane == 0) s.put(i, max_f, max_j);
 		__syncwarp();
 		if (hf < max_f) hf = max_f, hi = i, a_hi = ai;
 	}
 }
+
+__global__ void __launch_bounds__(SEG_WARPS * 32) chain_seg_fill_kernel(const int32_t *list, int n_list, int pool, const int64_t *a_off, const int32_t *cnt,
+                                                                       const uint64_t *a_all, Par par, int32_t *f_all, int32_t *p_all, int32_t *t_all,
+                                                                       int32_t *seg_all, int32_t *stat)
+{
+	extern __shared__ uint64_t sa[];
+	int32_t *sf = (int32_t*)(sa + pool);
+	int16_t *sp = (int16_t*)(sf + pool), *stt = sp + pool;
+	__shared__ int32_t s_nseg, s_next, s_one;
+	if ((int)blockIdx.x >= n_list) return;
+	const int prob = list[blockIdx.x], warp = threadIdx.x >> 5, lane = threadIdx.x & 31;
+	const int64_t base = a_off[prob];
+	const int32_t n = cnt ? cnt[prob] : (int32_t)(a_off[prob + 1] - base);
+	const uint64_t *a = a_all + base;
+	int32_t *f = f_all + base, *p = p_all + base, *t = t_all + base, *seg = seg_all + base;
+	if (threadIdx.x == 0) s_nseg = 0, s_next = 0, s_one = 0;
+	__syncthreads();
+	int32_t one = 0;
+	for (int32_t i = threadIdx.x; i < n; i += blockDim.x) {
+		const uint64_t ai = __ldg(a + i);
+		if (i > 0 && !isolated(par, __ldg(a + i - 1), ai)) continue;
+		if (i + 1 >= n || isolated(par, ai, __ldg(a + i + 1))) f[i] = par.kmer, p[i] = -1, ++one;
+		else seg[atomicAdd(&s_nseg, 1)] = i;
+	}
+	if (stat && one) atomicAdd(&s_one, one);
+	__syncthreads();
+	const int32_t n_seg = s_nseg;
+	const bool whole = n <= pool;
+	const int32_t slice = pool / SEG_WARPS, wbase = warp * slice;
+	int32_t longest = 0;
+	for (;;) {
+		int32_t k0 = 0;
+		if (lane == 0) k0 = atomicAdd(&s_next, 32);
+		k0 = __shfl_sync(0xffffffffu, k0, 0);
+		if (k0 >= n_seg) break;
+		int32_t s0 = 0, len = 0;
+		if (k0 + lane < n_seg) {
+			s0 = seg[k0 + lane], len = 1;
+		}
+		uint64_t w[SEG_SHORT + 1];
+#pragma unroll
+		for (int q = 0; q <= SEG_SHORT; ++q) w[q] = len && s0 + q < n ? __ldg(a + s0 + q) : 0;
+#pragma unroll
+		for (int q = 1; q <= SEG_SHORT; ++q)
+			if (len == q && s0 + q < n && !isolated(par, w[q - 1], w[q])) len = q + 1;
+		if (len > 1 && len <= SEG_SHORT) {
+			const int32_t o = whole ? s0 : wbase + lane * SEG_SHORT;
+#pragma unroll
+			for (int q = 0; q < SEG_SHORT; ++q)
+				if (q < len) sa[o + q] = w[q];
+			fill_serial(par, sa + o, len, sf + o, sp + o, stt + o);
+			for (int32_t q = 0; q < len; ++q) f[s0 + q] = sf[o + q], p[s0 + q] = sp[o + q] < 0 ? -1 : s0 + sp[o + q];
+			longest = len > longest ? len : longest;
+		}
+		__syncwarp();
+		for (uint32_t lm = __ballot_sync(0xffffffffu, len > SEG_SHORT); lm; lm &= lm - 1) {
+			const int32_t s0l = __shfl_sync(0xffffffffu, s0, __ffs(lm) - 1);
+			int32_t L = SEG_SHORT + 1;
+			for (;;) {
+				const int32_t q = s0l + L + lane;
+				const uint32_t m = __ballot_sync(0xffffffffu, q >= n || isolated(par, __ldg(a + q - 1), __ldg(a + q)));
+				if (m) { L += __ffs(m) - 1; break; }
+				L += 32;
+			}
+			longest = L > longest ? L : longest;
+			if (whole || L <= slice) {
+				const int32_t o = whole ? s0l : wbase;
+				for (int32_t q = lane; q < L; q += 32) sa[o + q] = __ldg(a + s0l + q), stt[o + q] = 0;
+				__syncwarp();
+				fill_warp(par, L, SegShared{ sa + o, sf + o, sp + o, stt + o, f + s0l, p + s0l, s0l }, lane);
+			} else {
+				for (int32_t q = lane; q < L; q += 32) __stcg(t + s0l + q, 0);
+				__syncwarp();
+				fill_warp(par, L, SegGlobal{ a + s0l, f + s0l, p + s0l, t + s0l, s0l }, lane);
+			}
+			__syncwarp();
+		}
+	}
+	if (stat) {
+		for (int d = 16; d; d >>= 1) { const int32_t o = __shfl_xor_sync(0xffffffffu, longest, d); longest = o > longest ? o : longest; }
+		if (lane == 0 && longest > 0) atomicMax(stat + 1, longest);
+		__syncthreads();
+		if (threadIdx.x == 0) {
+			atomicAdd(stat, s_nseg + s_one);
+			if (s_one) atomicMax(stat + 1, 1);
+		}
+	}
+}
+
+constexpr int BT_BATCH = 4;
 
 struct WarpSortScratch { uint32_t cnt[256]; uint32_t head[256]; uint32_t tail[256]; int top; };
 
@@ -226,125 +271,23 @@
 	for (int32_t k = lane; k < n_v; k += 32) t[v[k]] = 1;
 	__syncwarp();
 	int32_t o = 0;
-	for (int32_t i0 = 0; i0 < n; i0 += 32) {
-		const int32_t i = i0 + lane;
-		const bool keep = i < n && t[i] != 0;
-		const uint32_t m = __ballot_sync(0xffffffffu, keep);
-		if (keep) b[o + __popc(m & ((1u << lane) - 1u))] = a[i];
-		o += __popc(m);
+	for (int32_t i0 = 0; i0 < n; i0 += 32 * BT_BATCH) {
+		uint64_t av[BT_BATCH];
+		bool kv[BT_BATCH];
+#pragma unroll
+		for (int k = 0; k < BT_BATCH; ++k) {
+			const int32_t i = i0 + 32 * k + lane;
+			kv[k] = i < n && t[i] != 0;
+			av[k] = kv[k] ? a[i] : 0;
+		}
+#pragma unroll
+		for (int k = 0; k < BT_BATCH; ++k) {
+			const uint32_t m = __ballot_sync(0xffffffffu, kv[k]);
+			if (kv[k]) b[o + __popc(m & ((1u << lane) - 1u))] = av[k];
+			o += __popc(m);
+		}
 	}
 	return o;
-}
-
-__global__ void __launch_bounds__(32) chain_smem_kernel(const int32_t *list, int n_list, int cap, const int64_t *a_off, const int32_t *cnt, const uint64_t *a_all,
-                                                       Par par, int32_t *v_all, FlagRange<uint64_t> *stack_all, uint64_t *u_all, uint64_t *b_all,
-                                                       int32_t *n_u_out, int32_t *n_b_out, int resort)
-{
-	extern __shared__ uint64_t zs[];
-	__shared__ WarpSortScratch ws;
-	if ((int)blockIdx.x >= n_list) return;
-	const int prob = list[blockIdx.x], lane = threadIdx.x;
-	const int64_t base = a_off[prob];
-	const int32_t n = cnt ? cnt[prob] : (int32_t)(a_off[prob + 1] - base);
-	const uint64_t *a = a_all + base;
-	int32_t *f = (int32_t*)(zs + cap);
-	int16_t *p = (int16_t*)(f + cap), *t = p + cap;
-	for (int32_t i = lane; i < n; i += 32) t[i] = 0;
-	__syncwarp();
-	AnchorBlocks ab;
-	ab.init(a, n, lane);
-	int32_t st = 0, hi = -1, hf = 0;
-	uint64_t a_hi = 0;
-	for (int32_t i = 0; i < n; ++i) {
-		if (i && (i & 31) == 0) ab.enter(a, n, i, lane);
-		{
-			const uint64_t mine = ab.cur;
-			uint64_t left = __shfl_up_sync(0xffffffffu, mine, 1);
-			const uint64_t last_prev = __shfl_sync(0xffffffffu, ab.prev, 31);
-			if (lane == 0) left = last_prev;
-			const int32_t idx = ab.i0 + lane;
-			const bool iso = idx < n && (idx == 0 || (((int64_t)(mine >> 32) - (int64_t)(left >> 32)) << par.bbit) > par.max_dist_x);
-			const uint32_t m = __ballot_sync(0xffffffffu, iso) >> (i & 31);
-			const int run = ~m ? __ffs(~m) - 1 : 32;
-			if (run > 0) {
-				if (lane >= (i & 31) && lane < (i & 31) + run) f[idx] = par.kmer, p[idx] = -1;
-				__syncwarp();
-				i += run - 1;
-				st = i, hf = par.kmer, hi = i, a_hi = __shfl_sync(0xffffffffu, mine, i & 31);
-				continue;
-			}
-		}
-		const uint64_t ai = __shfl_sync(0xffffffffu, ab.cur, i & 31);
-		const int64_t xi = (int64_t)(ai >> 32);
-		while (st < i && ((xi - (int64_t)(ab.at(a, st) >> 32)) << par.bbit) > par.max_dist_x) ++st;
-		int32_t max_f = par.kmer, max_j = -1, n_skip = 0;
-		if (hi >= 0 && hi >= st) {
-			const int32_t sc = hf + pair_score(par, ai, a_hi);
-			if (sc > max_f) max_f = sc, max_j = hi;
-		} else hf = 0, hi = -1;
-		if (i - st > par.max_iter) st = i - par.max_iter;
-		for (int32_t jb = i - 1; jb >= st; jb -= 32) {
-			const int32_t j = jb - lane;
-			bool ok = j >= st;
-			int32_t sc = INT32_MIN, pj = -1;
-			uint64_t aj = 0;
-			if (jb == i - 1) aj = ab.near(j);
-			else if (ok) aj = a[j];
-			if (ok) {
-				sc = pair_score(par, ai, aj);
-				ok = sc != INT32_MIN;
-				if (ok) sc += f[j], pj = p[j];
-			}
-			if (ok && pj >= 0) t[pj] = (int16_t)i;
-			__syncwarp();
-			const bool marked = ok && t[j] == (int16_t)i;
-			int32_t pm = ok ? sc : INT32_MIN;
-#pragma unroll
-			for (int d = 1; d < 32; d <<= 1) {
-				const int32_t o = __shfl_up_sync(0xffffffffu, pm, d);
-				if (lane >= d) pm = pm > o ? pm : o;
-			}
-			int32_t before = __shfl_up_sync(0xffffffffu, pm, 1);
-			if (lane == 0) before = INT32_MIN;
-			before = before > max_f ? before : max_f;
-			const bool rec = ok && sc > before;
-			const uint32_t R = __ballot_sync(0xffffffffu, rec), S = __ballot_sync(0xffffffffu, ok && !rec && marked);
-			const int brk = resolve_chunk(R, S, par.max_skip, n_skip);
-			const uint32_t Rb = brk >= 32 ? R : (R & ((1u << brk) - 1u));
-			if (Rb) {
-				const int top = 31 - __clz(Rb);
-				max_f = __shfl_sync(0xffffffffu, sc, top), max_j = jb - top;
-			}
-			if (brk < 32) break;
-		}
-		if (lane == 0) f[i] = max_f, p[i] = (int16_t)max_j;
-		__syncwarp();
-		if (hf < max_f) hf = max_f, hi = i, a_hi = ai;
-	}
-	int32_t n_z = 0;
-	for (int32_t i0 = 0; i0 < n; i0 += 32) {
-		const int32_t i = i0 + lane;
-		const bool keep = i < n && f[i] >= par.min_sc;
-		if (i < n) t[i] = 0;
-		const uint32_t m = __ballot_sync(0xffffffffu, keep);
-		if (keep) zs[n_z + __popc(m & ((1u << lane) - 1u))] = (uint64_t)(uint32_t)f[i] << 32 | (uint32_t)i;
-		n_z += __popc(m);
-	}
-	__syncwarp();
-	int32_t n_u = 0, n_b = 0;
-	FlagRange<uint64_t> *stack = stack_all + (int64_t)prob * CHAIN_STACK;
-	flag_sort_warp(zs, n_z, [](const uint64_t &e) { return rec_key(e); }, stack, &ws, lane);
-	int32_t n_v = 0;
-	if (lane == 0 && n > 0) n_u = peel_chains<int16_t, true, int32_t, int16_t>(par, n_z, f, p, t, v_all + base, zs, stack, u_all + base, &n_v);
-	n_u = __shfl_sync(0xffffffffu, n_u, 0), n_v = __shfl_sync(0xffffffffu, n_v, 0);
-	__syncwarp();
-	if (resort) n_b = keep_filter_warp(n, n_v, v_all + base, t, a, b_all + base, lane);
-	else {
-		if (n > 0) compact_chains(n_u, a, f, v_all + base, zs, stack, u_all + base, b_all + base, &n_b, lane, 32, [] { __syncwarp(); });
-		__syncwarp();
-		n_b = __shfl_sync(0xffffffffu, n_b, 0);
-	}
-	if (lane == 0) n_u_out[prob] = n_u, n_b_out[prob] = n_b;
 }
 
 __global__ void __launch_bounds__(32) chain_bt_smem_kernel(const int32_t *list, int n_list, int cap, const int64_t *a_off, const int32_t *cnt, const uint64_t *a_all,
@@ -364,15 +307,23 @@
 	const int32_t *pg = p_all + base;
 	int32_t n_z = 0;
 	bool wide = false;
-	for (int32_t i0 = 0; i0 < n; i0 += 32) {
-		const int32_t i = i0 + lane;
-		const int32_t fi = i < n ? fg[i] : 0;
-		const bool keep = i < n && fi >= par.min_sc;
-		if (i < n) ts[i] = 0, ps[i] = (int16_t)pg[i], fs[i] = (uint16_t)fi;
-		wide |= fi > 65535;
-		const uint32_t m = __ballot_sync(0xffffffffu, keep);
-		if (keep) zs[n_z + __popc(m & ((1u << lane) - 1u))] = (uint64_t)(uint32_t)fi << 32 | (uint32_t)i;
-		n_z += __popc(m);
+	for (int32_t i0 = 0; i0 < n; i0 += 32 * BT_BATCH) {
+		int32_t fv[BT_BATCH], pv[BT_BATCH];
+#pragma unroll
+		for (int k = 0; k < BT_BATCH; ++k) {
+			const int32_t i = i0 + 32 * k + lane;
+			fv[k] = i < n ? fg[i] : 0, pv[k] = i < n ? pg[i] : 0;
+		}
+#pragma unroll
+		for (int k = 0; k < BT_BATCH; ++k) {
+			const int32_t i = i0 + 32 * k + lane, fi = fv[k];
+			const bool keep = i < n && fi >= par.min_sc;
+			if (i < n) ts[i] = 0, ps[i] = (int16_t)pv[k], fs[i] = (uint16_t)fi;
+			wide |= fi > 65535;
+			const uint32_t m = __ballot_sync(0xffffffffu, keep);
+			if (keep) zs[n_z + __popc(m & ((1u << lane) - 1u))] = (uint64_t)(uint32_t)fi << 32 | (uint32_t)i;
+			n_z += __popc(m);
+		}
 	}
 	wide = __any_sync(0xffffffffu, wide);
 	__syncwarp();
@@ -439,20 +390,14 @@
 	if (lane == 0) n_u_out[prob] = n_u, n_b_out[prob] = n_b;
 }
 
-void chain_launch_fill(cudaStream_t st, const int32_t *list, const int64_t *a_off, const int32_t *cnt, const uint64_t *a, int n_prob, const Par &par, int32_t *f, int32_t *p,
-                       int32_t *t)
-{
-	if (n_prob > 0) chain_fill_kernel<<<(n_prob + CHAIN_WARPS - 1) / CHAIN_WARPS, CHAIN_WARPS * 32, 0, st>>>(list, a_off, cnt, a, n_prob, par, f, p, t);
-}
-
-void chain_launch_smem(cudaStream_t st, const int32_t *list, int n_list, int cap, const int64_t *a_off, const int32_t *cnt, const uint64_t *a, const Par &par, int32_t *v,
-                       void *stack, uint64_t *u, uint64_t *b, int32_t *n_u, int32_t *n_b, int resort)
+void chain_launch_fill(cudaStream_t st, const int32_t *list, int n_list, int pool, const int64_t *a_off, const int32_t *cnt, const uint64_t *a, const Par &par,
+                       int32_t *f, int32_t *p, int32_t *t, int32_t *seg, int32_t *stat)
 {
 	if (n_list <= 0) return;
-	const int smem = cap * 16 + 16;
+	const int smem = pool * 16;
 	static SmemLimit lim;
-	lim.raise(chain_smem_kernel, smem);
-	chain_smem_kernel<<<n_list, 32, smem, st>>>(list, n_list, cap, a_off, cnt, a, par, v, (FlagRange<uint64_t>*)stack, u, b, n_u, n_b, resort);
+	lim.raise(chain_seg_fill_kernel, smem);
+	chain_seg_fill_kernel<<<n_list, SEG_WARPS * 32, smem, st>>>(list, n_list, pool, a_off, cnt, a, par, f, p, t, seg, stat);
 }
 
 void chain_launch_bt_smem(cudaStream_t st, const int32_t *list, int n_list, int cap, const int64_t *a_off, const int32_t *cnt, const uint64_t *a, const Par &par,
diff --git a/miniprot_b200/csrc/cuda/stage_host.cu b/miniprot_b200/csrc/cuda/stage_host.cu
--- a/miniprot_b200/csrc/cuda/stage_host.cu
+++ b/miniprot_b200/csrc/cuda/stage_host.cu
@@ -1,5 +1,6 @@
 #include <algorithm>
 #include <numeric>
+#include <string>
 #include "ctx.hpp"
 #include "stages_dev.hpp"
 #include "chain_dev.hpp"
@@ -89,8 +90,8 @@
 	return room;
 }
 
-static void chain_problems(mpb_ctx_s *ctx, int n_prob, const std::vector<int64_t> &h_off, const int64_t *d_off, uint64_t *d_a, const chn::Par *pre, const chn::Par &mainp,
-                           std::vector<int32_t> &n_u, std::vector<int32_t> &n_b, std::vector<uint64_t> &u, std::vector<uint64_t> &bb)
+static void chain_problems(mpb_ctx_s *ctx, const char *what, int n_prob, const std::vector<int64_t> &h_off, const int64_t *d_off, uint64_t *d_a, const chn::Par *pre,
+                           const chn::Par &mainp, std::vector<int32_t> &n_u, std::vector<int32_t> &n_b, std::vector<uint64_t> &u, std::vector<uint64_t> &bb)
 {
 	cudaStream_t st = ctx->stream;
 	const size_t N = (size_t)h_off[(size_t)n_prob];
@@ -106,7 +107,7 @@
 	void *stack = cs.stack;
 	static const int NC = 11;
 	static const int caps[NC] = { 2048, 3072, 4096, 5120, 6144, 7168, 8192, 10240, 12288, 14000, 16384 };
-	static const int fused_max = getenv("MPB_CHAIN_FUSED_MAX") ? atoi(getenv("MPB_CHAIN_FUSED_MAX")) : 2048;
+	static const bool trace = getenv("MPB_TRACE") != 0;
 	std::vector<int32_t> lists[NC + 1], flat, sizes((size_t)n_prob);
 	size_t lfirst[NC + 1];
 	for (int i = 0; i < n_prob; ++i) sizes[(size_t)i] = (int32_t)(h_off[(size_t)i + 1] - h_off[(size_t)i]);
@@ -123,38 +124,66 @@
 		MPB_CUDA_OK(cudaMemcpyAsync(d_list, flat.data(), sizeof(int32_t) * flat.size(), cudaMemcpyHostToDevice, st));
 	};
 	classify();
-	auto chain_once = [&](const int32_t *cnt, const uint64_t *in, const chn::Par &par, uint64_t *uo, uint64_t *bo, int32_t *nuo, int32_t *nbo, int resort) {
+	auto chain_once = [&](const char *what, const int32_t *cnt, const uint64_t *in, const chn::Par &par, uint64_t *uo, uint64_t *bo, int32_t *nuo, int32_t *nbo, int resort) {
+		cudaEvent_t tev[NC + 1][3] = {};
+		int32_t *d_stat = 0;
+		if (trace) {
+			MPB_CUDA_OK(cudaMallocAsync((void**)&d_stat, sizeof(int32_t) * 2 * (NC + 1), st));
+			MPB_CUDA_OK(cudaMemsetAsync(d_stat, 0, sizeof(int32_t) * 2 * (NC + 1), st));
+		}
 		MPB_CUDA_OK(cudaEventRecord(ctx->ev_fork, st));
 		for (int c = NC; c >= 0; --c) {
 			if (lists[c].empty()) continue;
 			cudaStream_t ss = ctx->side[c];
 			const int32_t *lst = d_list + lfirst[c];
 			const int nl = (int)lists[c].size();
+			int32_t largest = 0;
+			for (int32_t i : lists[c]) largest = std::max(largest, sizes[(size_t)i]);
+			const int cap = (std::max(largest, 1) + 31) & ~31, pool = std::min(cap, SEG_POOL);
 			MPB_CUDA_OK(cudaStreamWaitEvent(ss, ctx->ev_fork, 0));
-			if (c < NC && caps[c] <= fused_max) {
-				chain_launch_smem(ss, lst, nl, caps[c], d_off, cnt, in, par, v, stack, uo, bo, nuo, nbo, resort);
-				ctx->stats.kernel_launches += 1;
-			} else {
-				chain_launch_fill(ss, lst, d_off, cnt, in, nl, par, f, p, t);
-				if (c < NC) chain_launch_bt_smem(ss, lst, nl, caps[c], d_off, cnt, in, par, f, p, v, stack, uo, bo, nuo, nbo, resort);
-				else chain_launch_bt(ss, lst, nl, d_off, cnt, in, par, f, p, t, v, z, stack, uo, bo, nuo, nbo, resort);
-				ctx->stats.kernel_launches += 2;
-			}
+			if (trace) for (int k = 0; k < 3; ++k) MPB_CUDA_OK(cudaEventCreate(&tev[c][k]));
+			if (trace) MPB_CUDA_OK(cudaEventRecord(tev[c][0], ss));
+			chain_launch_fill(ss, lst, nl, pool, d_off, cnt, in, par, f, p, t, v, d_stat ? d_stat + 2 * c : 0);
+			if (trace) MPB_CUDA_OK(cudaEventRecord(tev[c][1], ss));
+			if (c < NC) chain_launch_bt_smem(ss, lst, nl, cap, d_off, cnt, in, par, f, p, v, stack, uo, bo, nuo, nbo, resort);
+			else chain_launch_bt(ss, lst, nl, d_off, cnt, in, par, f, p, t, v, z, stack, uo, bo, nuo, nbo, resort);
+			if (trace) MPB_CUDA_OK(cudaEventRecord(tev[c][2], ss));
+			ctx->stats.kernel_launches += 2;
 			MPB_CUDA_OK(cudaEventRecord(ctx->ev_join[c], ss));
 			MPB_CUDA_OK(cudaStreamWaitEvent(st, ctx->ev_join[c], 0));
 		}
+		if (!trace) return;
+		int32_t h_stat[2 * (NC + 1)];
+		MPB_CUDA_OK(cudaMemcpyAsync(h_stat, d_stat, sizeof(h_stat), cudaMemcpyDeviceToHost, st));
+		MPB_CUDA_OK(cudaStreamSynchronize(st));
+		MPB_CUDA_OK(cudaFreeAsync(d_stat, st));
+		std::string line;
+		for (int c = 0; c <= NC; ++c) {
+			if (lists[c].empty()) continue;
+			int32_t largest = 0;
+			for (int32_t i : lists[c]) largest = std::max(largest, sizes[(size_t)i]);
+			float ms_fill = 0, ms_bt = 0;
+			cudaEventElapsedTime(&ms_fill, tev[c][0], tev[c][1]);
+			cudaEventElapsedTime(&ms_bt, tev[c][1], tev[c][2]);
+			char buf[256];
+			snprintf(buf, sizeof(buf), " | class %d (<= %d): %zu problems, largest %d, fill %.3f ms, backtrack %.3f ms, %d segments, longest %d", c,
+			         c < NC ? caps[c] : -1, lists[c].size(), largest, ms_fill, ms_bt, h_stat[2 * c], h_stat[2 * c + 1]);
+			line += buf;
+			for (int k = 0; k < 3; ++k) cudaEventDestroy(tev[c][k]);
+		}
+		fprintf(stderr, "[mpb-trace] chain %s: %d problems%s\n", what, n_prob, line.c_str());
 	};
 	ctx->time_begin();
 	const uint64_t *in = d_a;
 	const int32_t *cnt = 0;
 	if (pre) {
-		chain_once(0, d_a, *pre, du, db, d_nu, d_nb, 1);
+		chain_once("pre", 0, d_a, *pre, du, db, d_nu, d_nb, 1);
 		in = db, cnt = d_nb;
 		MPB_CUDA_OK(cudaMemcpyAsync(sizes.data(), d_nb, sizeof(int32_t) * (size_t)n_prob, cudaMemcpyDeviceToHost, st));
 		MPB_CUDA_OK(cudaStreamSynchronize(st));
 		classify();
 	}
-	chain_once(cnt, in, mainp, du2, db2, d_nu2, d_nb2, 0);
+	chain_once(what, cnt, in, mainp, du2, db2, d_nu2, d_nb2, 0);
 	MPB_CUDA_OK(cudaMemcpyAsync(n_u.data(), d_nu2, sizeof(int32_t) * (size_t)n_prob, cudaMemcpyDeviceToHost, st));
 	MPB_CUDA_OK(cudaMemcpyAsync(n_b.data(), d_nb2, sizeof(int32_t) * (size_t)n_prob, cudaMemcpyDeviceToHost, st));
 	MPB_CUDA_OK(cudaStreamSynchronize(st));
@@ -186,7 +215,7 @@
 	MPB_CUDA_OK(cudaMemcpyAsync(ctx->b_c[1].p, a, sizeof(uint64_t) * N, cudaMemcpyHostToDevice, st));
 	MPB_CUDA_OK(cudaMemcpyAsync(ctx->b_c[7].p, off.data(), sizeof(int64_t) * off.size(), cudaMemcpyHostToDevice, st));
 	ctx->stats.h2d_bytes += (int64_t)(sizeof(uint64_t) * N);
-	chain_problems(ctx, n_prob, off, ctx->b_c[7].as<int64_t>(), ctx->b_c[1].as<uint64_t>(), 0, chn::normalise(par), n_u, n_b, u, bb);
+	chain_problems(ctx, "batch", n_prob, off, ctx->b_c[7].as<int64_t>(), ctx->b_c[1].as<uint64_t>(), 0, chn::normalise(par), n_u, n_b, u, bb);
 }
 
 template <class F>
@@ -276,7 +305,7 @@
 	const chn::Par mainp = chain_par(opt->max_intron, opt->max_gap, opt->bw, opt, opt->min_chn_cnt, opt->min_chn_sc, mi->opt.kmer, mi->opt.bbit);
 	std::vector<int32_t> n_u, n_b;
 	std::vector<uint64_t> u, bb;
-	chain_problems(ctx, n, a_off, d_a_off, d_a, (!(opt->flag & MP_F_NO_PRE_CHAIN) && spl) ? &pre : 0, mainp, n_u, n_b, u, bb);
+	chain_problems(ctx, "main", n, a_off, d_a_off, d_a, (!(opt->flag & MP_F_NO_PRE_CHAIN) && spl) ? &pre : 0, mainp, n_u, n_b, u, bb);
 	for (int q = 0; q < n; ++q) {
 		const size_t g = (size_t)(q0 + q);
 		out.u_off[g + 1] = out.u_off[g] + n_u[(size_t)q], out.a_off[g + 1] = out.a_off[g] + n_b[(size_t)q];
@@ -517,7 +546,7 @@
 		seg_sort_u64(ctx, st, d_a, d_tmp, n, a_off.data(), a_off.data() + 1);
 		ctx->stats.ms_refine += ctx->time_end();
 		ctx->stats.kernel_launches += 2;
-		chain_problems(ctx, n, a_off, d_a_off, d_a, 0, par, n_u, n_b, u, bb);
+		chain_problems(ctx, "refine", n, a_off, d_a_off, d_a, 0, par, n_u, n_b, u, bb);
 		size_t uo = 0, bo = 0;
 		for (int j = 0; j < n; ++j) {
 			const int32_t nu = n_u[(size_t)j];
```

Result: faster. 22090 (median of 6 runs) (+11.1%).
